# Walter0807/MotionBERT

Measured on AMD Instinct MI355X. Metric: clips/sec [B,243,17,3] DSTformer fwd+bwd, higher is better.
Workload: dtype bf16; 1 GPU; MotionBERT full DSTformer (dim_feat 512, depth 5, 8 heads, mlp_ratio 2) train step: fwd + bwd + AdamW, 64 clips/GPU x T=243 x J=17, random-init weights, pose loss (mpjpe + 0.5 n_mpjpe + 20 velocity, fused kernel), one-launch flat AdamW; global_batch=64, frames=243, parallelism=dp1

## Files before the change

include/mbx.h:

```cpp
#ifndef MBX_H
#define MBX_H
#include <stddef.h>
#include <stdint.h>

#ifdef __cplusplus
extern "C" {
#endif

enum mbx_dtype {
    MBX_F32 = 0,
    MBX_BF16 = 1,
    MBX_BF16_LO = 2
};

enum mbx_epilogue {
    MBX_EPI_STORE = 0,
    MBX_EPI_GELU  = 1,
    MBX_EPI_RESID = 2,
    MBX_EPI_TANH  = 3,
    MBX_EPI_DGELU = 4,
    MBX_EPI_LNBWD = 5,
    MBX_EPI_LNBWD_T = 9,
    MBX_EPI_GELU_D = 10,
    MBX_EPI_MULAUX = 11
};

enum mbx_attn_mode {
    MBX_ATTN_SPATIAL  = 0,
    MBX_ATTN_TEMPORAL = 1
};

const char* mbx_last_error(void);
int mbx_version(void);

int mbx_prep_weights(const int64_t* desc, int n_desc, int max_n, int max_k, int dtype, void* stream);

int mbx_embed_fwd(const float* x, const float* w, const float* b, const float* pos, const float* temp,
                  float* h, int B, int T, int J, int Din, int C, void* stream);
size_t mbx_embed_bwd_ws(int T, int J, int Din, int C);
int mbx_embed_bwd(const float* dh, const float* x, const float* w, float* dw, float* db, float* dpos,
                  float* dtemp, float* dx, int B, int T, int J, int Din, int C, void* ws, void* stream);
int mbx_embed_bwd_pair(const void* dh_a, const void* dh_b, const float* x, const float* w, float* dw, float* db, float* dpos,
                       float* dtemp, float* dx, int B, int T, int J, int Din, int C, void* ws, void* stream);

int mbx_layernorm_fwd(const float* x, const float* gamma, const float* beta, float eps, void* y,
                      float* mean, float* rstd, int M, int C, int dtype, void* stream);
size_t mbx_layernorm_bwd_ws(int C);
int mbx_layernorm_bwd(const void* dy, const float* x, const float* mean, const float* rstd, const float* gamma,
                      const float* dres, const float* extra, float* dx, void* dx_t, float* dgamma, float* dbeta,
                      int M, int C, int dtype, void* ws, void* stream);
int mbx_layernorm_bwd_planes(const float* dy, const float* x, const float* mean, const float* rstd, const float* gamma, const float* dres,
                             const float* extra, float* dx, void* dx_hi, void* dx_lo, float* dgamma, float* dbeta, int M, int C,
                             void* ws, void* stream);

int mbx_gemm_nt(const void* a, const void* w, const float* bias, int epilogue, void* out_t, void* out2_t,
                float* out_f, const float* resid, const void* aux_t, int M, int N, int K, int dtype, void* stream);
size_t mbx_gemm_tn_ws(int M, int N, int K);
int mbx_gemm_tn(const void* dy, const void* a, float* dw, float* db, int M, int N, int K, int dtype,
                void* ws, void* stream);

int mbx_fold_norm_weights(const int64_t* desc, int n_desc, int max_n, int max_k, void* stream);
int mbx_gemm_nt_dgelu_stats(const void* a, const void* w, void* out_t, const void* aux_t, const float* bias_f,
                            const float* rsum, float* part, int M, int N, int K, void* stream);
int mbx_gemm_nt_gelu_d(const void* a, const void* w, const float* bias, void* out_d, void* out_g, int M, int N, int K, void* stream);
int mbx_gemm_nt_mul(const void* a, const void* w, const void* aux, void* out, int M, int N, int K, void* stream);
int mbx_lnbwd_rowc(const float* part, int nb, const float* rstd, float* rowc, int M, int C, void* stream);
int mbx_gemm_nt_lnbwd(const void* a, const void* w, const void* xhat, const float* rowc, const float* dres,
                      const float* extra, float* dx, void* dx_t, int M, int N, int K, void* stream);
int mbx_gemm_nt_lnbwd_t(const void* a, const void* w, const void* xhat, const float* rowc, const void* dres_t,
                        const float* extra, float* dx, void* dx_t, int M, int N, int K, void* stream);
size_t mbx_unfold_norm_grads_ws(int N, int K);
int mbx_unfold_norm_grads(float* dw, const float* db, const float* w, const float* gamma, const float* beta,
                          float* dgamma, float* dbeta, int N, int K, void* ws, void* stream);

size_t mbx_mlp_pack_bytes(int C, int hidden);
int mbx_mlp_pack_weights(const void* w1, const void* w2, void* packed, int C, int hidden, void* stream);
int mbx_mlp_fused_fwd(const void* a, int raw_in, const void* packed, const float* b1, const float* b2, const float* rsum,
                      const float* resid, float* y, void* y_t, float eps, float* mean, float* rstd, int M, int C, int hidden,
                      void* stream);
size_t mbx_proj_mlp_pack_bytes(int C, int hidden);
int mbx_proj_mlp_pack_weights(const void* wp, const void* w1, const void* w2, void* packed, int C, int hidden, void* stream);
int mbx_proj_mlp_fused_fwd(const void* o, const void* packed, const float* bp, const float* b1, const float* b2, const float* rsum,
                           const float* resid, float* y, float eps, int M, int C, int hidden, void* stream);

size_t mbx_rows_pack_bytes(int N, int K);
int mbx_rows_pack_nk(const void* w, void* packed, int N, int K, void* stream);
int mbx_rows_gemm_nk(const void* a, const void* packed, const float* bias, const float* rsum, const float* mean, const float* rstd,
                     void* out, int M, int N, int K, void* stream);
int mbx_rows_gemm_nk_ln(const float* x, const void* packed, const float* bias, const float* rsum, float eps, void* out, int M, int N,
                        int K, void* stream);

int mbx_gelu_fwd(const void* u, void* g, size_t n, int dtype, void* stream);

int mbx_split_bf16(const float* x, void* hi, void* lo, size_t n, void* stream);
int mbx_gemm_nt_x3(const void* a_hi, const void* a_lo, const void* w_hi, const void* w_lo, const float* bias, int epilogue,
                   float* out_t, float* out2_t, float* out_f, const float* resid, const float* aux_t, int M, int N, int K,
                   void* stream);
int mbx_gemm_nt_x3p(const void* a_hi, const void* a_lo, const void* w_hi, const void* w_lo, const float* bias, int epilogue,
                    float* out_t, void* pl_hi, void* pl_lo, const float* aux_t, int M, int N, int K, void* stream);
int mbx_layernorm_fwd_planes(const float* x, const float* gamma, const float* beta, float eps, void* y_hi, void* y_lo, float* mean,
                             float* rstd, int M, int C, void* stream);
size_t mbx_gemm_tn_x3_workspace(int M, int N, int K);
int mbx_gemm_tn_x3(const void* dy_hi, const void* dy_lo, const void* a_hi, const void* a_lo, float* dw, float* db, int M,
                   int N, int K, void* ws, void* stream);

int mbx_attn_fwd(const void* qkv, void* o, float* lse, int B, int T, int J, int H, int hd, float scale,
                 int mode, int dtype, void* stream);
int mbx_attn_fwd_drop(const void* qkv, void* o, float* lse, int B, int T, int J, int H, int hd, float scale,
                      int mode, int dtype, float p, uint64_t seed, void* stream);
int mbx_attn_bwd(const void* qkv, const void* o, const void* d_o, const float* lse, void* dqkv, int B, int T,
                 int J, int H, int hd, float scale, int mode, int dtype, void* stream);
int mbx_attn_bwd_drop(const void* qkv, const void* o, const void* d_o, const float* lse, void* dqkv, int B, int T,
                      int J, int H, int hd, float scale, int mode, int dtype, float p, uint64_t seed, void* stream);
int mbx_attn_bwd_planes(const void* qkv, const void* o, const void* d_o, const float* lse, void* dqkv_hi, void* dqkv_lo, int B, int T,
                        int J, int H, int hd, float scale, int mode, float p, uint64_t seed, void* stream);
int mbx_attn_bwd_stats(const void* qkv, const void* o, const void* d_o, const float* lse, void* dqkv, const float* bias_f,
                       const float* rsum, float* part, int B, int T, int J, int H, int hd, float scale, int mode, void* stream);

int mbx_fuse_fwd(const float* x_st, const float* x_ts, const float* w, const float* b, float* out, float* alpha,
                 int M, int C, void* stream);
int mbx_fuse_ln_fwd(const float* x_st, const float* x_ts, const float* w, const float* b, float* out, float* alpha,
                    const float* g1, const float* b1, void* xn1, const float* g2, const float* b2, void* xn2, float eps,
                    float* mean, float* rstd, int M, int C, int dtype, void* stream);
size_t mbx_fuse_bwd_ws(int C);
int mbx_fuse_bwd(const float* dh, const float* x_st, const float* x_ts, const float* alpha, const float* w,
                 float* d_st, float* d_ts, void* d_st_t, void* d_ts_t, float* dw, float* db, int M, int C,
                 int dtype, void* ws, void* stream);
int mbx_fuse_bwd_pair(const void* dh_a, const void* dh_b, const float* x_st, const float* x_ts, const float* alpha, const float* w,
                      void* d_st_t, void* d_ts_t, float* dw, float* db, int M, int C, void* ws, void* stream);
int mbx_average(const float* x_st, const float* x_ts, float* out, size_t n, void* stream);
int mbx_average_bwd(const float* dh, float* d_st, float* d_ts, void* d_st_t, void* d_ts_t, size_t n, int dtype,
                    void* stream);

int mbx_head_fwd(const float* rep, const float* w, const float* b, float* out, int M, int R, int Dout, void* stream);
size_t mbx_head_bwd_ws(int R, int Dout);
int mbx_head_bwd(const float* dout, const float* rep, const float* w, void* dpre_t, float* dw, float* db,
                 int M, int R, int Dout, int dtype, void* ws, void* stream);
int mbx_tanh_bwd(const float* drep, const float* rep, void* dpre_t, size_t n, int dtype, void* stream);

size_t mbx_pose_loss_ws(int B, int T);
int mbx_pose_loss(const float* pred, const float* gt, float lambda_scale, float lambda_velocity, float* losses, float* dpred,
                  float grad_scale, int B, int T, int J, void* ws, void* stream);
size_t mbx_pose_loss_full_ws(int B, int T);
int mbx_pose_loss_full(const float* pred, const float* gt, float lambda_scale, float lambda_velocity, float lambda_lv, float lambda_lg,
                       float lambda_a, float lambda_av, float* losses, float* dpred, float grad_scale, int B, int T, int J, void* ws,
                       void* stream);
size_t mbx_loss_2d_weighted_ws(int B, int T);
int mbx_loss_2d_weighted(const float* pred, const float* target, int target_stride, const float* conf, int conf_stride, float* loss,
                         float* dpred, float grad_scale, int B, int T, int J, void* ws, void* stream);
int mbx_adamw_step(float* p, const float* g, float* m, float* v, size_t n, float* state, float beta1, float beta2, float eps,
                   float weight_decay, int tick, void* stream);

int mbx_pool_rep_fwd(const float* rep, float* pooled, int N, int Mp, int T, int J, int R, float p, uint64_t seed, void* stream);
int mbx_tanh_pool_bwd(const float* dpooled, const float* rep, void* dpre_t, int N, int Mp, int T, int J, int R, float p,
                      uint64_t seed, int dtype, void* stream);

int mbx_dropout(const void* x, void* y, size_t n, float p, uint64_t seed, int dtype, void* stream);
int mbx_residual_drop(float* y, const float* x, size_t rows, int C, int rows_per_sample, float p, uint64_t seed, float p_path,
                      uint64_t seed_path, void* stream);
int mbx_grad_drop(const float* dy, void* dy_t, size_t rows, int C, int rows_per_sample, float p, uint64_t seed, float p_path,
                  uint64_t seed_path, int dtype, void* stream);

int mbx_augment2d(const float* x, float* y, int B, int T, int J, int Cin, const float* noise_mean, const float* noise_std,
                  const float* noise_weight, float uniform_range, float jitter_std, float d2c_a, float d2c_b, float d2c_m,
                  float d2c_s, float mask_ratio, float mask_T_ratio, int flags, uint64_t seed, void* stream);
int mbx_embed_fwd_tta(const float* x, const int* perm, const float* w, const float* b, const float* pos, const float* temp,
                      float* h, int B, int T, int J, int Din, int C, void* stream);
int mbx_flip_average(const float* out2, const int* perm, float* out, int B, int T, int J, int D, void* stream);

int mbx_pose_errors(const float* pred, const float* gt, const float* hw, const float* factor, const float* x, int x_channels, int rootrel,
                    int gt_2d, double* e1, double* e2, int N, int T, int J, void* stream);
size_t mbx_eval_reduce_ws(int F, int A);
int mbx_eval_reduce(const double* e1, const double* e2, int n_err, const int* row_ptr, int n_row_ptr, const int* slots, int nnz,
                    const int* action, int F, int A, double* per_action, double* summary, int* count, void* ws, void* stream);

size_t mbx_rows_n_pack_bytes(int N, int K);
int mbx_rows_n_pack_many(const int64_t* desc, int n_desc, int N, int max_k, void* stream);
int mbx_rows_lnbwd_t(const void* dy, const void* packed, const void* xhat, const float* rstd, const void* dres_t, void* dx_t, int M,
                     int N, int K, void* stream);
int mbx_rows_resid_ln(const void* a, const void* packed, const float* bias, const float* resid, float* y, void* xhat, float* mean,
                      float* rstd, float eps, int M, int N, int K, void* stream);

size_t mbx_supcon_loss_ws(int A, int D);
int mbx_supcon_loss(const float* feat, const int* labels, int bsz, int n_views, int D, float temperature, float base_temperature,
                    int normalize, float grad_scale, float* loss, float* dfeat, void* ws, void* stream);
int mbx_nn_cosine(const float* anchors, const int* anchor_labels, int M, const float* test, const int* test_labels, int N, int D,
                  int* pred_label, float* best_sim, long long* hits, void* stream);

int mbx_rot6d_theta_fwd(const float* x6, float* rotmat, float* aa, int M, void* stream);
int mbx_rot6d_theta_bwd(const float* x6, const float* drotmat, const float* daa, float* dx6, int M, void* stream);
size_t mbx_mesh_param_loss_ws(int F);
// ... 93 lines not shown
```

motionbert_amd/csrc/elementwise.hip:

```cpp
#include "mbx_common.h"

static thread_local char g_err[512] = "";
int mbx_set_error(const char* fmt, ...) {
    va_list ap;
    va_start(ap, fmt);
    vsnprintf(g_err, sizeof(g_err), fmt, ap);
    va_end(ap);
    return 1;
}
extern "C" const char* mbx_last_error(void) { return g_err; }

#include <atomic>
static std::atomic<uintptr_t> g_lds_key[512];
static std::atomic<size_t> g_lds_size[512];
int mbx_set_dyn_lds(const void* kernel, size_t bytes, const char* who) {
    if (bytes > 160 * 1024) return mbx_set_error("%s: needs %zu bytes of LDS (> 160 KiB)", who, bytes);
    int dev = 0;
    if (hipGetDevice(&dev) != hipSuccess) dev = 0;
    const uintptr_t key = (reinterpret_cast<uintptr_t>(kernel) << 6) ^ (uintptr_t)(dev + 1);
    int slot = (int)((key * 0x9E3779B97F4A7C15ull) >> 55);
    for (int probe = 0; probe < 512; ++probe, slot = (slot + 1) & 511) {
        uintptr_t k = g_lds_key[slot].load(std::memory_order_acquire);
        if (k == 0 && g_lds_key[slot].compare_exchange_strong(k, key, std::memory_order_acq_rel)) k = key;
        if (k != key) continue;
        if (g_lds_size[slot].load(std::memory_order_acquire) >= bytes) return 0;
        const hipError_t e = hipFuncSetAttribute(kernel, hipFuncAttributeMaxDynamicSharedMemorySize, (int)bytes);
        if (e != hipSuccess) return mbx_set_error("%s: hipFuncSetAttribute(%zu): %s", who, bytes, hipGetErrorString(e));
        size_t cur = g_lds_size[slot].load(std::memory_order_relaxed);
        while (cur < bytes && !g_lds_size[slot].compare_exchange_weak(cur, bytes, std::memory_order_release)) { }
        return 0;
    }
    const hipError_t e = hipFuncSetAttribute(kernel, hipFuncAttributeMaxDynamicSharedMemorySize, (int)bytes);
    return e == hipSuccess ? 0 : mbx_set_error("%s: hipFuncSetAttribute(%zu): %s", who, bytes, hipGetErrorString(e));
}
static std::atomic<int> g_cus[64];
int mbx_cu_count() {
    int dev = 0;
    if (hipGetDevice(&dev) != hipSuccess || dev < 0 || dev >= 64) dev = 0;
    int c = g_cus[dev].load(std::memory_order_relaxed);
    if (c > 0) return c;
    if (hipDeviceGetAttribute(&c, hipDeviceAttributeMultiprocessorCount, dev) != hipSuccess || c <= 0) c = 256;
    g_cus[dev].store(c, std::memory_order_relaxed);
    return c;
}
extern "C" int mbx_version(void) { return 210; }

static inline int clamp_grid(size_t want, int cap) { return (int)(want < (size_t)cap ? (want ? want : 1) : (size_t)cap); }

__device__ __forceinline__ float4 ld4(const float* p) { return *reinterpret_cast<const float4*>(p); }
template <int CL>
__global__ __launch_bounds__(256) void colsum4_kernel(const float* __restrict__ part, int nparts, size_t stride, int ncols,
                                                      float* __restrict__ out0, float* __restrict__ out1, int split) {
    constexpr int PLW = 64 / CL, PL = 4 * PLW;
    __shared__ float4 red[PL][CL];
    const int lane = threadIdx.x & 63, wave = threadIdx.x >> 6;
    const int cl = lane % CL, pl = wave * PLW + lane / CL;
    const int c = (blockIdx.x * CL + cl) * 4;
    float4 a0 = make_float4(0.f, 0.f, 0.f, 0.f), a1 = a0, a2 = a0, a3 = a0;
    if (c < ncols) {
        const float* p = part + c;
        int i = pl;
        for (; i + 3 * PL < nparts; i += 4 * PL) {
            const float4 v0 = ld4(p + (size_t)i * stride), v1 = ld4(p + (size_t)(i + PL) * stride);
            const float4 v2 = ld4(p + (size_t)(i + 2 * PL) * stride), v3 = ld4(p + (size_t)(i + 3 * PL) * stride);
            a0 += v0; a1 += v1; a2 += v2; a3 += v3;
        }
        for (; i < nparts; i += PL) a0 += ld4(p + (size_t)i * stride);
    }
    red[pl][cl] = (a0 + a1) + (a2 + a3);
    __syncthreads();
    if (pl == 0 && c < ncols) {
        float4 t = red[0][cl];
#pragma unroll
        for (int q = 1; q < PL; ++q) t += red[q][cl];
        float* o = c < split ? out0 + c : out1 + (c - split);
        if ((reinterpret_cast<uintptr_t>(o) & 15) == 0) {
            *reinterpret_cast<float4*>(o) = t;
        } else {
            o[0] = t.x; o[1] = t.y; o[2] = t.z; o[3] = t.w;
        }
    }
}
__global__ __launch_bounds__(256) void colsum_kernel(const float* __restrict__ part, int nparts, int stride, int col0,
                                                     int ncols, float* __restrict__ out) {
    __shared__ float red[4][64];
    const int cl = threadIdx.x & 63, grp = threadIdx.x >> 6;
    const int c = blockIdx.x * 64 + cl;
    float s0 = 0.f, s1 = 0.f, s2 = 0.f, s3 = 0.f;
    if (c < ncols) {
        const float* p = part + col0 + c;
        int i = grp;
        for (; i + 12 < nparts; i += 16) {
            s0 += p[(size_t)i * stride];
            s1 += p[(size_t)(i + 4) * stride];
            s2 += p[(size_t)(i + 8) * stride];
            s3 += p[(size_t)(i + 12) * stride];
        }
        for (; i < nparts; i += 4) s0 += p[(size_t)i * stride];
    }
    red[grp][cl] = (s0 + s1) + (s2 + s3);
    __syncthreads();
    if (grp == 0 && c < ncols) out[c] = (red[0][cl] + red[1][cl]) + (red[2][cl] + red[3][cl]);
}
static int launch_colsum2(const float* part, int nparts, int stride, int col0, int ncols, float* out0, float* out1, int split,
                          hipStream_t s) {
    const bool vec = ncols % 4 == 0 && col0 % 4 == 0 && stride % 4 == 0 && split % 4 == 0 &&
                     (reinterpret_cast<uintptr_t>(part + col0) & 15) == 0;
    if (!vec) {
        hipLaunchKernelGGL(colsum_kernel, dim3((split + 63) / 64), dim3(256), 0, s, part, nparts, stride, col0, split, out0);
        if (ncols > split)
            hipLaunchKernelGGL(colsum_kernel, dim3((ncols - split + 63) / 64), dim3(256), 0, s, part, nparts, stride, col0 + split,
                               ncols - split, out1);
    } else if (ncols / 4 >= 64 * 512) {
        hipLaunchKernelGGL(colsum4_kernel<64>, dim3((ncols / 4 + 63) / 64), dim3(256), 0, s, part + col0, nparts, (size_t)stride, ncols,
                           out0, out1, split);
    } else {
        hipLaunchKernelGGL(colsum4_kernel<16>, dim3((ncols / 4 + 15) / 16), dim3(256), 0, s, part + col0, nparts, (size_t)stride, ncols,
                           out0, out1, split);
    }
    MBX_LAUNCH_CHECK("colsum");
    return 0;
}
int mbx_launch_colsum(const float* part, int nparts, int stride, int col0, int ncols, float* out, hipStream_t s) {
    return launch_colsum2(part, nparts, stride, col0, ncols, out, nullptr, ncols, s);
}

struct BfLo {};
template <> struct Cvt<BfLo> {
    static __device__ __forceinline__ bf16_t from_f(float v) { return f2bf(v - bf2f(f2bf(v))); }
};
template <typename T> struct PrepOut { typedef T type; };
template <> struct PrepOut<BfLo> { typedef bf16_t type; };
template <typename TT>
__global__ __launch_bounds__(256) void prep_weights_kernel(const int64_t* __restrict__ desc) {
    typedef typename PrepOut<TT>::type T;
    __shared__ float tile[32][33];
    const int64_t* d = desc + (size_t)blockIdx.y * 5;
    const float* src = reinterpret_cast<const float*>(d[0]);
    T* dst_n = reinterpret_cast<T*>(d[1]);
    T* dst_t = reinterpret_cast<T*>(d[2]);
    const int N = (int)d[3], K = (int)d[4];
    const int tk = (K + 31) / 32, tn = (N + 31) / 32;
    if ((int)blockIdx.x >= tk * tn) return;
    const int n0 = (blockIdx.x / tk) * 32, k0 = (blockIdx.x % tk) * 32;
    const int cx = threadIdx.x & 31, ry = threadIdx.x >> 5;
#pragma unroll
    for (int i = 0; i < 4; ++i) {
        const int r = ry + 8 * i;
        float v = 0.f;
        if (n0 + r < N && k0 + cx < K) {
            v = src[(size_t)(n0 + r) * K + k0 + cx];
            if (dst_n) dst_n[(size_t)(n0 + r) * K + k0 + cx] = Cvt<TT>::from_f(v);
        }
        tile[r][cx] = v;
    }
    __syncthreads();
    if (dst_t) {
#pragma unroll
        for (int i = 0; i < 4; ++i) {
            const int r = ry + 8 * i;
            if (k0 + r < K && n0 + cx < N) dst_t[(size_t)(k0 + r) * N + n0 + cx] = Cvt<TT>::from_f(tile[cx][r]);
        }
    }
}
extern "C" int mbx_prep_weights(const int64_t* desc, int n_desc, int max_n, int max_k, int dtype, void* stream) {
    MBX_CHECK_ARG(desc && n_desc > 0 && max_n > 0 && max_k > 0, "prep_weights: bad arguments");
    dim3 grid(((max_n + 31) / 32) * ((max_k + 31) / 32), n_desc);
    if (dtype == MBX_BF16)
        hipLaunchKernelGGL(prep_weights_kernel<bf16_t>, grid, dim3(256), 0, (hipStream_t)stream, desc);
    else if (dtype == MBX_F32)
        hipLaunchKernelGGL(prep_weights_kernel<float>, grid, dim3(256), 0, (hipStream_t)stream, desc);
    else if (dtype == MBX_BF16_LO)
        hipLaunchKernelGGL(prep_weights_kernel<BfLo>, grid, dim3(256), 0, (hipStream_t)stream, desc);
    else
        return mbx_set_error("prep_weights: unknown dtype %d", dtype);
    MBX_LAUNCH_CHECK("prep_weights");
    return 0;
}

template <typename T>
__global__ __launch_bounds__(256) void gelu_fwd_kernel(const T* __restrict__ u, T* __restrict__ g, size_t n4) {
    for (size_t i = (size_t)blockIdx.x * 256 + threadIdx.x; i < n4; i += (size_t)gridDim.x * 256) {
        float v[4];
        load4<T>(u + i * 4, v);
#pragma unroll
        for (int e = 0; e < 4; ++e) v[e] = gelu_erf(v[e]);
        store4<T>(g + i * 4, v);
    }
}
extern "C" int mbx_gelu_fwd(const void* u, void* g, size_t n, int dtype, void* stream) {
    MBX_CHECK_ARG(u && g && n % 4 == 0, "gelu_fwd: bad arguments");
    if (n == 0) return 0;
    const int grid = clamp_grid((n / 4 + 255) / 256, 256 * 16);
    if (dtype == MBX_BF16)
        hipLaunchKernelGGL(gelu_fwd_kernel<bf16_t>, dim3(grid), dim3(256), 0, (hipStream_t)stream, (const bf16_t*)u, (bf16_t*)g, n / 4);
    else if (dtype == MBX_F32)
        hipLaunchKernelGGL(gelu_fwd_kernel<float>, dim3(grid), dim3(256), 0, (hipStream_t)stream, (const float*)u, (float*)g, n / 4);
    else
        return mbx_set_error("gelu_fwd: unknown dtype %d", dtype);
    MBX_LAUNCH_CHECK("gelu_fwd");
    return 0;
}

__global__ __launch_bounds__(256) void split_bf16_kernel(const float* __restrict__ x, bf16_t* __restrict__ hi, bf16_t* __restrict__ lo,
                                                        size_t n4) {
    for (size_t idx = (size_t)blockIdx.x * 256 + threadIdx.x; idx < n4; idx += (size_t)gridDim.x * 256) {
        float v[4], h[4], l[4];
        load4<float>(x + idx * 4, v);
#pragma unroll
        for (int e = 0; e < 4; ++e) { h[e] = bf2f(f2bf(v[e])); l[e] = v[e] - h[e]; }
        store4<bf16_t>(hi + idx * 4, h);
        store4<bf16_t>(lo + idx * 4, l);
    }
}
extern "C" int mbx_split_bf16(const float* x, void* hi, void* lo, size_t n, void* stream) {
    MBX_CHECK_ARG(x && hi && lo, "split_bf16: null pointer");
    MBX_CHECK_ARG(n % 4 == 0, "split_bf16: n %% 4 != 0");
    if (n == 0) return 0;
    const int grid = clamp_grid((n / 4 + 255) / 256, 256 * 16);
    hipLaunchKernelGGL(split_bf16_kernel, dim3(grid), dim3(256), 0, (hipStream_t)stream, x, (bf16_t*)hi, (bf16_t*)lo, n / 4);
    MBX_LAUNCH_CHECK("split_bf16");
    return 0;
}

__global__ __launch_bounds__(256) void embed_fwd_kernel(const float* __restrict__ x, const float* __restrict__ w,
                                                        const float* __restrict__ b, const float* __restrict__ pos,
                                                        const float* __restrict__ temp, float* __restrict__ h, int M,
                                                        int T, int J, int Din, int C) {
    const int c4n = C >> 2;
    const size_t total = (size_t)M * c4n;
    for (size_t idx = (size_t)blockIdx.x * 256 + threadIdx.x; idx < total; idx += (size_t)gridDim.x * 256) {
        const int m = (int)(idx / c4n), c = (int)(idx % c4n) * 4;
        const int j = m % J, t = (m / J) % T;
        const float4 bb = *reinterpret_cast<const float4*>(b + c);
        const float4 pp = *reinterpret_cast<const float4*>(pos + (size_t)j * C + c);
        const float4 tt = *reinterpret_cast<const float4*>(temp + (size_t)t * C + c);
        float a0 = 0.f, a1 = 0.f, a2 = 0.f, a3 = 0.f;
        for (int k = 0; k < Din; ++k) {
            const float xv = x[(size_t)m * Din + k];
            a0 = fmaf(xv, w[(size_t)(c + 0) * Din + k], a0);
            a1 = fmaf(xv, w[(size_t)(c + 1) * Din + k], a1);
            a2 = fmaf(xv, w[(size_t)(c + 2) * Din + k], a2);
            a3 = fmaf(xv, w[(size_t)(c + 3) * Din + k], a3);
        }
        *reinterpret_cast<float4*>(h + (size_t)m * C + c) =
            make_float4(((a0 + bb.x) + pp.x) + tt.x, ((a1 + bb.y) + pp.y) + tt.y, ((a2 + bb.z) + pp.z) + tt.z,
                        ((a3 + bb.w) + pp.w) + tt.w);
    }
}
#define EMBF_MAXDIN 4
__global__ __launch_bounds__(256) void embed_fwd_rows_kernel(const float* __restrict__ x, const float* __restrict__ w,
                                                             const float* __restrict__ b, const float* __restrict__ pos,
                                                             const float* __restrict__ temp, float* __restrict__ h, int M,
                                                             int T, int J, int Din, int C, int chunk) {
    const int c4n = C >> 2, rpp = 256 / c4n;
    const int c = ((int)threadIdx.x % c4n) * 4, rsub = (int)threadIdx.x / c4n;
    float wv[4][EMBF_MAXDIN];
#pragma unroll
    for (int e = 0; e < 4; ++e)
#pragma unroll
        for (int k = 0; k < EMBF_MAXDIN; ++k) wv[e][k] = k < Din ? w[(size_t)(c + e) * Din + k] : 0.f;
    const float4 bb = *reinterpret_cast<const float4*>(b + c);
    const int end = min(M, ((int)blockIdx.x + 1) * chunk);
    int m = (int)blockIdx.x * chunk + rsub;
    int j = m % J, t = (m / J) % T;
    for (; m < end; m += 4 * rpp) {
        float xv[4][EMBF_MAXDIN];
        float4 pp[4], tt[4];
        int jj = j, tq = t;
#pragma unroll
        for (int u = 0; u < 4; ++u) {
            const int mu = min(m + u * rpp, M - 1);
#pragma unroll
            for (int k = 0; k < EMBF_MAXDIN; ++k) xv[u][k] = k < Din ? x[(size_t)mu * Din + k] : 0.f;
            pp[u] = *reinterpret_cast<const float4*>(pos + (size_t)jj * C + c);
            tt[u] = *reinterpret_cast<const float4*>(temp + (size_t)tq * C + c);
            jj += rpp;
            if (jj >= J) { jj -= J; tq = tq + 1 == T ? 0 : tq + 1; }
        }
#pragma unroll
        for (int u = 0; u < 4; ++u) {
            float a[4] = {0.f, 0.f, 0.f, 0.f};
#pragma unroll
            for (int k = 0; k < EMBF_MAXDIN; ++k)
                if (k < Din) {
#pragma unroll
                    for (int e = 0; e < 4; ++e) a[e] = fmaf(xv[u][k], wv[e][k], a[e]);
                }
            if (m + u * rpp < end)
                *reinterpret_cast<float4*>(h + (size_t)(m + u * rpp) * C + c) =
                    make_float4(((a[0] + bb.x) + pp[u].x) + tt[u].x, ((a[1] + bb.y) + pp[u].y) + tt[u].y,
                                ((a[2] + bb.z) + pp[u].z) + tt[u].z, ((a[3] + bb.w) + pp[u].w) + tt[u].w);
        }
        j = jj;
        t = tq;
    }
}
extern "C" int mbx_embed_fwd(const float* x, const float* w, const float* b, const float* pos, const float* temp,
                             float* h, int B, int T, int J, int Din, int C, void* stream) {
    MBX_CHECK_ARG(x && w && b && pos && temp && h, "embed_fwd: null pointer");
    MBX_CHECK_ARG(B > 0 && T > 0 && J > 0 && Din > 0 && C > 0 && C % 4 == 0, "embed_fwd: bad shape (C %% 4 != 0?)");
    const int M = B * T * J;
    const int c4n = C / 4;
    if (c4n >= 16 && c4n <= 256 && (c4n & (c4n - 1)) == 0 && Din <= EMBF_MAXDIN && 256 / c4n <= J) {
        const int rpp = 256 / c4n;
        const int blocks = clamp_grid((M + 4 * rpp - 1) / (4 * rpp), 256 * 8);
        int chunk = (M + blocks - 1) / blocks;
        chunk = ((chunk + 4 * rpp - 1) / (4 * rpp)) * (4 * rpp);
        const int grid = (M + chunk - 1) / chunk;
        hipLaunchKernelGGL(embed_fwd_rows_kernel, dim3(grid), dim3(256), 0, (hipStream_t)stream, x, w, b, pos, temp, h, M, T, J, Din, C, chunk);
    } else {
        const int grid = clamp_grid(((size_t)M * (C / 4) + 255) / 256, 256 * 16);
        hipLaunchKernelGGL(embed_fwd_kernel, dim3(grid), dim3(256), 0, (hipStream_t)stream, x, w, b, pos, temp, h, M, T, J, Din, C);
    }
    MBX_LAUNCH_CHECK("embed_fwd");
    return 0;
}

template <bool TTA>
__global__ __launch_bounds__(256) void embed_fwd_ragged_kernel(const float* __restrict__ x, const int* __restrict__ perm,
                                                               const float* __restrict__ w, const float* __restrict__ b,
                                                               const float* __restrict__ pos, const float* __restrict__ temp,
                                                               const int* __restrict__ frame_t, float* __restrict__ h, int F, int J,
                                                               int Din, int C, int n_temp) {
    const int c4n = C >> 2;
    const size_t rows = (size_t)(TTA ? 2 : 1) * F * J, total = rows * c4n;
    for (size_t idx = (size_t)blockIdx.x * 256 + threadIdx.x; idx < total; idx += (size_t)gridDim.x * 256) {
        const size_t mo = idx / c4n;
        const int c = (int)(idx % c4n) * 4;
        const int j = (int)(mo % J);
        size_t f = mo / J;
        const bool flip = TTA && f >= (size_t)F;
        if (flip) f -= F;
        const int t = frame_t[f];
        if (t < 0 || t >= n_temp) continue;
        const size_t ms = f * J + (flip ? perm[j] : j);
        const float4 bb = *reinterpret_cast<const float4*>(b + c);
        const float4 pp = *reinterpret_cast<const float4*>(pos + (size_t)j * C + c);
        const float4 tt = *reinterpret_cast<const float4*>(temp + (size_t)t * C + c);
        float a0 = 0.f, a1 = 0.f, a2 = 0.f, a3 = 0.f;
        for (int k = 0; k < Din; ++k) {
            float xv = x[ms * Din + k];
            if (flip && k == 0) xv = -xv;
            a0 = fmaf(xv, w[(size_t)(c + 0) * Din + k], a0);
            a1 = fmaf(xv, w[(size_t)(c + 1) * Din + k], a1);
            a2 = fmaf(xv, w[(size_t)(c + 2) * Din + k], a2);
            a3 = fmaf(xv, w[(size_t)(c + 3) * Din + k], a3);
        }
        *reinterpret_cast<float4*>(h + mo * C + c) =
            make_float4(((a0 + bb.x) + pp.x) + tt.x, ((a1 + bb.y) + pp.y) + tt.y, ((a2 + bb.z) + pp.z) + tt.z, ((a3 + bb.w) + pp.w) + tt.w);
    }
}
static int embed_fwd_ragged_impl(const char* who, const float* x, const int* perm, const float* w, const float* b, const float* pos,
                                 const float* temp, const int* frame_t, float* h, int F, int J, int Din, int C, int n_temp, bool tta,
                                 void* stream) {
    MBX_CHECK_ARG(x && w && b && pos && temp && frame_t && h && (!tta || perm), "%s: null pointer", who);
    MBX_CHECK_ARG(F > 0 && J > 0 && Din > 0 && C > 0 && C % 4 == 0 && n_temp > 0, "%s: bad shape (C %% 4 != 0?)", who);
    const int grid = clamp_grid(((size_t)(tta ? 2 : 1) * F * J * (C / 4) + 255) / 256, 256 * 16);
    if (tta)
        hipLaunchKernelGGL(embed_fwd_ragged_kernel<true>, dim3(grid), dim3(256), 0, (hipStream_t)stream, x, perm, w, b, pos, temp, frame_t, h, F, J,
                           Din, C, n_temp);
    else
        hipLaunchKernelGGL(embed_fwd_ragged_kernel<false>, dim3(grid), dim3(256), 0, (hipStream_t)stream, x, perm, w, b, pos, temp, frame_t, h, F, J,
                           Din, C, n_temp);
    MBX_LAUNCH_CHECK(who);
    return 0;
}
extern "C" int mbx_embed_fwd_ragged(const float* x, const float* w, const float* b, const float* pos, const float* temp, const int* frame_t,
                                    float* h, int F, int J, int Din, int C, int n_temp, void* stream) {
    return embed_fwd_ragged_impl("embed_fwd_ragged", x, nullptr, w, b, pos, temp, frame_t, h, F, J, Din, C, n_temp, false, stream);
}
extern "C" int mbx_embed_fwd_tta_ragged(const float* x, const int* perm, const float* w, const float* b, const float* pos, const float* temp,
                                        const int* frame_t, float* h, int F, int J, int Din, int C, int n_temp, void* stream) {
    return embed_fwd_ragged_impl("embed_fwd_tta_ragged", x, perm, w, b, pos, temp, frame_t, h, F, J, Din, C, n_temp, true, stream);
}

#define EMB_MAXDIN 4
__device__ __forceinline__ float4 embed_dh4(const float* __restrict__ dh, const bf16_t* __restrict__ dh_a, const bf16_t* __restrict__ dh_b, size_t o) {
    if (dh_a == nullptr) return *reinterpret_cast<const float4*>(dh + o);
    float u[4], v[4];
    load4<bf16_t>(dh_a + o, u);
    load4<bf16_t>(dh_b + o, v);
    return make_float4(u[0] + v[0], u[1] + v[1], u[2] + v[2], u[3] + v[3]);
}
__global__ __launch_bounds__(256) void embed_bwd_kernel(const float* __restrict__ dh, const float* __restrict__ x,
                                                        float* __restrict__ dtemp, float* __restrict__ part, int B, int T,
                                                        int J, int Din, int C, const bf16_t* __restrict__ dh_a = nullptr,
                                                        const bf16_t* __restrict__ dh_b = nullptr) {
    __shared__ float4 red[256][1 + EMB_MAXDIN];
    const int t = blockIdx.x;
    const int stride = J * C + C * Din + C;
    float* prow = part + (size_t)t * stride;
    const int nq = C / 4, ns = max(256 / nq, 1);
    for (int q0 = 0; q0 < nq; q0 += 256) {
        const int q = q0 + (int)threadIdx.x % min(nq, 256), sl = (int)threadIdx.x / min(nq, 256);
        const bool act = q < nq && sl < ns;
        const int c = q * 4;
        float4 at = make_float4(0.f, 0.f, 0.f, 0.f), aw[EMB_MAXDIN];
#pragma unroll
        for (int k = 0; k < EMB_MAXDIN; ++k) aw[k] = make_float4(0.f, 0.f, 0.f, 0.f);
        for (int j = 0; j < J; ++j) {
            float4 ap = make_float4(0.f, 0.f, 0.f, 0.f);
            if (act) {
                for (int b0 = sl; b0 < B; b0 += 8 * ns) {
                    float4 g[8];
#pragma unroll
                    for (int u = 0; u < 8; ++u) {
                        const int b = min(b0 + u * ns, B - 1);
                        g[u] = embed_dh4(dh, dh_a, dh_b, (((size_t)b * T + t) * J + j) * C + c);
                    }
#pragma unroll
                    for (int u = 0; u < 8; ++u) {
                        const int b = b0 + u * ns;
                        const float on = b < B ? 1.f : 0.f;
                        const size_t m = ((size_t)min(b, B - 1) * T + t) * J + j;
                        ap.x = fmaf(on, g[u].x, ap.x); ap.y = fmaf(on, g[u].y, ap.y); ap.z = fmaf(on, g[u].z, ap.z); ap.w = fmaf(on, g[u].w, ap.w);
#pragma unroll
                        for (int k = 0; k < EMB_MAXDIN; ++k)
                            if (k < Din) {
                                const float xv = on * x[m * Din + k];
                                aw[k].x = fmaf(g[u].x, xv, aw[k].x); aw[k].y = fmaf(g[u].y, xv, aw[k].y);
                                aw[k].z = fmaf(g[u].z, xv, aw[k].z); aw[k].w = fmaf(g[u].w, xv, aw[k].w);
                            }
                    }
                }
            }
            red[threadIdx.x][0] = ap;
            __syncthreads();
            if (act && sl == 0) {
                for (int s2 = 1; s2 < ns; ++s2) {
                    const float4 o = red[threadIdx.x + s2 * nq][0];
                    ap.x += o.x; ap.y += o.y; ap.z += o.z; ap.w += o.w;
                }
                *reinterpret_cast<float4*>(prow + (size_t)j * C + c) = ap;
                at.x += ap.x; at.y += ap.y; at.z += ap.z; at.w += ap.w;
            }
            __syncthreads();
        }
#pragma unroll
        for (int k = 0; k < EMB_MAXDIN; ++k) red[threadIdx.x][1 + k] = aw[k];
        __syncthreads();
        if (act && sl == 0) {
            *reinterpret_cast<float4*>(dtemp + (size_t)t * C + c) = at;
            *reinterpret_cast<float4*>(prow + (size_t)J * C + (size_t)C * Din + c) = at;
#pragma unroll
            for (int k = 0; k < EMB_MAXDIN; ++k)
                if (k < Din) {
                    float4 w4 = aw[k];
                    for (int s2 = 1; s2 < ns; ++s2) {
                        const float4 o = red[threadIdx.x + s2 * nq][1 + k];
                        w4.x += o.x; w4.y += o.y; w4.z += o.z; w4.w += o.w;
                    }
                    float* d = prow + (size_t)J * C + (size_t)c * Din + k;
                    d[0] = w4.x; d[Din] = w4.y; d[2 * Din] = w4.z; d[3 * Din] = w4.w;
                }
        }
        __syncthreads();
    }
}
__global__ __launch_bounds__(256) void embed_bwd_dx_kernel(const float* __restrict__ dh, const float* __restrict__ w,
                                                           float* __restrict__ dx, int M, int Din, int C,
                                                           const bf16_t* __restrict__ dh_a = nullptr, const bf16_t* __restrict__ dh_b = nullptr) {
    const int lane = threadIdx.x & 63;
    for (int m = blockIdx.x * 4 + (threadIdx.x >> 6); m < M; m += gridDim.x * 4) {
        float a[EMB_MAXDIN] = {0.f, 0.f, 0.f, 0.f};
        for (int c = lane; c < C; c += 64) {
            const float g = dh_a == nullptr ? dh[(size_t)m * C + c] : bf2f(dh_a[(size_t)m * C + c]) + bf2f(dh_b[(size_t)m * C + c]);
#pragma unroll
            for (int k = 0; k < EMB_MAXDIN; ++k)
                if (k < Din) a[k] = fmaf(g, w[(size_t)c * Din + k], a[k]);
        }
#pragma unroll
        for (int k = 0; k < EMB_MAXDIN; ++k) {
            const float s = wave_sum(a[k]);
            if (lane == 0 && k < Din) dx[(size_t)m * Din + k] = s;
        }
    }
}
extern "C" size_t mbx_embed_bwd_ws(int T, int J, int Din, int C) { return (size_t)T * ((size_t)J * C + (size_t)C * Din + C) * sizeof(float); }
static int launch_embed_bwd(const float* dh, const bf16_t* dh_a, const bf16_t* dh_b, const float* x, const float* w, float* dw, float* db,
                            float* dpos, float* dtemp, float* dx, int B, int T, int J, int Din, int C, void* ws, void* stream) {
    MBX_CHECK_ARG((dh || (dh_a && dh_b)) && x && w && dw && db && dpos && dtemp && ws, "embed_bwd: null pointer");
    MBX_CHECK_ARG(Din <= EMB_MAXDIN, "embed_bwd: dim_in %d > %d unsupported", Din, EMB_MAXDIN);
    MBX_CHECK_ARG(B > 0 && T > 0 && J > 0 && C > 0 && C % 4 == 0, "embed_bwd: bad shape (C %% 4 != 0?)");
    hipStream_t s = (hipStream_t)stream;
    float* part = (float*)ws;
    const int stride = J * C + C * Din + C;
    hipLaunchKernelGGL(embed_bwd_kernel, dim3(T), dim3(256), 0, s, dh, x, dtemp, part, B, T, J, Din, C, dh_a, dh_b);
    MBX_LAUNCH_CHECK("embed_bwd");
    if (mbx_launch_colsum(part, T, stride, 0, J * C, dpos, s)) return 1;
    if (mbx_launch_colsum(part, T, stride, J * C, C * Din, dw, s)) return 1;
    if (mbx_launch_colsum(part, T, stride, J * C + C * Din, C, db, s)) return 1;
    if (dx) {
        const int M = B * T * J;
        hipLaunchKernelGGL(embed_bwd_dx_kernel, dim3(clamp_grid((M + 3) / 4, 2048)), dim3(256), 0, s, dh, w, dx, M, Din, C, dh_a, dh_b);
        MBX_LAUNCH_CHECK("embed_bwd_dx");
    }
    return 0;
}
extern "C" int mbx_embed_bwd(const float* dh, const float* x, const float* w, float* dw, float* db, float* dpos,
                             float* dtemp, float* dx, int B, int T, int J, int Din, int C, void* ws, void* stream) {
    MBX_CHECK_ARG(dh, "embed_bwd: null pointer");
    return launch_embed_bwd(dh, nullptr, nullptr, x, w, dw, db, dpos, dtemp, dx, B, T, J, Din, C, ws, stream);
}
extern "C" int mbx_embed_bwd_pair(const void* dh_a, const void* dh_b, const float* x, const float* w, float* dw, float* db, float* dpos,
                                  float* dtemp, float* dx, int B, int T, int J, int Din, int C, void* ws, void* stream) {
    MBX_CHECK_ARG(dh_a && dh_b, "embed_bwd_pair: null pointer");
    return launch_embed_bwd(nullptr, (const bf16_t*)dh_a, (const bf16_t*)dh_b, x, w, dw, db, dpos, dtemp, dx, B, T, J, Din, C, ws, stream);
}

#define ROW_LOOP(k) _Pragma("unroll") for (int k = 0; k < VPL; ++k)
#define ROW_C(k) (((k) * 64 + lane) * 4)

static inline int vpl_for(int C) { return C <= 256 ? 1 : C <= 512 ? 2 : C <= 1024 ? 4 : C <= 2048 ? 8 : 0; }
#define DISPATCH_VPL(vpl, ...)           \
    switch (vpl) {                       \
        case 1: { constexpr int VPL = 1; __VA_ARGS__; } break; \
        case 2: { constexpr int VPL = 2; __VA_ARGS__; } break; \
        case 4: { constexpr int VPL = 4; __VA_ARGS__; } break; \
        case 8: { constexpr int VPL = 8; __VA_ARGS__; } break; \
        default: return mbx_set_error("row kernel: channel count unsupported (need C %% 4 == 0 and C <= 2048)"); \
    }

#define LN_BLOCKS 1024
template <typename T> struct Raw4;
template <> struct Raw4<float> {
    typedef float4 type;
    static __device__ __forceinline__ void unpack(const float4& r, float (&v)[4]) { v[0] = r.x; v[1] = r.y; v[2] = r.z; v[3] = r.w; }
};
template <> struct Raw4<bf16_t> {
    typedef uint2 type;
    static __device__ __forceinline__ void unpack(const uint2& r, float (&v)[4]) {
        v[0] = __uint_as_float(r.x << 16); v[1] = __uint_as_float(r.x & 0xffff0000u);
        v[2] = __uint_as_float(r.y << 16); v[3] = __uint_as_float(r.y & 0xffff0000u);
    }
};
__device__ __forceinline__ void unpack4(const float4& r, float (&v)[4]) { v[0] = r.x; v[1] = r.y; v[2] = r.z; v[3] = r.w; }

template <int VPL, bool FULL>
__device__ __forceinline__ void ln_fwd_load(const float* __restrict__ x, int row, int C, int lane, float4 (&raw)[VPL]) {
    ROW_LOOP(k) {
        const int c = ROW_C(k);
        raw[k] = make_float4(0.f, 0.f, 0.f, 0.f);
        if (FULL || c < C) raw[k] = ld4(x + (size_t)row * C + c);
    }
}
template <typename T, int VPL, bool FULL>
__device__ __forceinline__ void ln_fwd_row(const float4 (&raw)[VPL], const float (&g)[VPL][4], const float (&bt)[VPL][4], float eps,
                                           float invC, T* __restrict__ y, float* __restrict__ mean, float* __restrict__ rstd,
                                           int row, int C, int lane, bf16_t* __restrict__ y_lo = nullptr) {
    float v[VPL][4];
    float s = 0.f;
    ROW_LOOP(k) {
        unpack4(raw[k], v[k]);
        s += (v[k][0] + v[k][1]) + (v[k][2] + v[k][3]);
    }
    const float mu = wave_sum(s) * invC;
    float q = 0.f;
    ROW_LOOP(k) {
        const int c = ROW_C(k);
        if (FULL || c < C) {
#pragma unroll
            for (int i = 0; i < 4; ++i) { v[k][i] -= mu; q = fmaf(v[k][i], v[k][i], q); }
        }
    }
    const float rs = 1.0f / sqrtf(wave_sum(q) * invC + eps);
    ROW_LOOP(k) {
        const int c = ROW_C(k);
        if (FULL || c < C) {
            float o[4];
#pragma unroll
            for (int i = 0; i < 4; ++i) o[i] = fmaf(v[k][i] * rs, g[k][i], bt[k][i]);
            if (sizeof(T) == 4 && y_lo)
                store4_planes(reinterpret_cast<bf16_t*>(y) + (size_t)row * C + c, y_lo + (size_t)row * C + c, o);
            else
                store4<T>(y + (size_t)row * C + c, o);
        }
    }
    if (lane == 0) { mean[row] = mu; rstd[row] = rs; }
}
template <typename T, int VPL, bool FULL>
__global__ __launch_bounds__(256) void ln_fwd_kernel(const float* __restrict__ x, const float* __restrict__ gamma,
                                                     const float* __restrict__ beta, float eps, T* __restrict__ y,
                                                     float* __restrict__ mean, float* __restrict__ rstd, int M, int C,
                                                     bf16_t* __restrict__ y_lo) {
    const int lane = threadIdx.x & 63;
    float g[VPL][4], bt[VPL][4];
    ROW_LOOP(k) {
        const int c = ROW_C(k);
#pragma unroll
        for (int i = 0; i < 4; ++i) { g[k][i] = 0.f; bt[k][i] = 0.f; }
        if (gamma == nullptr) {
#pragma unroll
            for (int i = 0; i < 4; ++i) g[k][i] = 1.f;
        } else if (FULL || c < C) { load4<float>(gamma + c, g[k]); load4<float>(beta + c, bt[k]); }
    }
    const float invC = 1.0f / (float)C;
    const int step = gridDim.x * 4;
    for (int row0 = blockIdx.x * 4 + (threadIdx.x >> 6); row0 < M; row0 += 2 * step) {
        const int row1 = row0 + step;
        float4 ra[VPL], rb[VPL];
        ln_fwd_load<VPL, FULL>(x, row0, C, lane, ra);
        if (row1 < M) ln_fwd_load<VPL, FULL>(x, row1, C, lane, rb);
        ln_fwd_row<T, VPL, FULL>(ra, g, bt, eps, invC, y, mean, rstd, row0, C, lane, y_lo);
        if (row1 < M) ln_fwd_row<T, VPL, FULL>(rb, g, bt, eps, invC, y, mean, rstd, row1, C, lane, y_lo);
    }
}
#define LN_FWD_LAUNCH(TT, FULLV)                                                                                             \
    DISPATCH_VPL(vpl, hipLaunchKernelGGL((ln_fwd_kernel<TT, VPL, FULLV>), dim3(grid), dim3(256), 0, s, x, gamma, beta, eps, (TT*)y, \
                                         mean, rstd, M, C, (bf16_t*)y_lo))
static int launch_layernorm_fwd(const float* x, const float* gamma, const float* beta, float eps, void* y, void* y_lo, float* mean,
                                float* rstd, int M, int C, int dtype, void* stream);
extern "C" int mbx_layernorm_fwd(const float* x, const float* gamma, const float* beta, float eps, void* y, float* mean,
                                 float* rstd, int M, int C, int dtype, void* stream) {
    return launch_layernorm_fwd(x, gamma, beta, eps, y, nullptr, mean, rstd, M, C, dtype, stream);
}
extern "C" int mbx_layernorm_fwd_planes(const float* x, const float* gamma, const float* beta, float eps, void* y_hi, void* y_lo,
                                        float* mean, float* rstd, int M, int C, void* stream) {
    MBX_CHECK_ARG(y_lo, "layernorm_fwd_planes: null pointer");
    return launch_layernorm_fwd(x, gamma, beta, eps, y_hi, y_lo, mean, rstd, M, C, MBX_F32, stream);
}
static int launch_layernorm_fwd(const float* x, const float* gamma, const float* beta, float eps, void* y, void* y_lo, float* mean,
                                float* rstd, int M, int C, int dtype, void* stream) {
    MBX_CHECK_ARG(x && y && mean && rstd, "layernorm_fwd: null pointer");
    MBX_CHECK_ARG((gamma && beta) || (!gamma && !beta), "layernorm_fwd: gamma and beta come together (both NULL = plain normalisation)");
    MBX_CHECK_ARG(M > 0 && C > 0 && C % 4 == 0, "layernorm_fwd: bad shape M=%d C=%d", M, C);
    MBX_CHECK_ARG(dtype == MBX_BF16 || dtype == MBX_F32, "layernorm_fwd: unknown dtype %d", dtype);
    const int grid = clamp_grid((M + 3) / 4, LN_BLOCKS);
    const int vpl = vpl_for(C);
    const bool full = vpl > 0 && C == vpl * 256;
    hipStream_t s = (hipStream_t)stream;
    if (dtype == MBX_BF16) {
        if (full) { LN_FWD_LAUNCH(bf16_t, true); } else { LN_FWD_LAUNCH(bf16_t, false); }
    } else {
        if (full) { LN_FWD_LAUNCH(float, true); } else { LN_FWD_LAUNCH(float, false); }
    }
    MBX_LAUNCH_CHECK("layernorm_fwd");
    return 0;
}

__device__ __forceinline__ void block_fold_store(const float* lds , int n, float* __restrict__ dst) {
    for (int i = threadIdx.x; i < n; i += 256) dst[i] = (lds[i] + lds[n + i]) + (lds[2 * n + i] + lds[3 * n + i]);
}

template <typename T, int VPL, bool FULL, bool RES>
__device__ __forceinline__ void ln_bwd_load(const T* __restrict__ dy, const float* __restrict__ x, const float* __restrict__ dres,
                                            const float* __restrict__ mean, const float* __restrict__ rstd, int row, int C, int lane,
                                            typename Raw4<T>::type (&rd)[VPL], float4 (&rx)[VPL], float4 (&rr)[VPL], float& mu,
                                            float& rs) {
    mu = mean[row];
    rs = rstd[row];
    ROW_LOOP(k) {
        const int c = ROW_C(k);
        if (FULL || c < C) {
            const size_t o = (size_t)row * C + c;
            rd[k] = *reinterpret_cast<const typename Raw4<T>::type*>(dy + o);
            rx[k] = ld4(x + o);
            if (RES) rr[k] = ld4(dres + o);
        }
    }
}
template <typename T, int VPL, bool FULL, bool RES>
__device__ __forceinline__ void ln_bwd_row(const typename Raw4<T>::type (&rd)[VPL], const float4 (&rx)[VPL], const float4 (&rr)[VPL],
                                           float mu, float rs, const float (&g)[VPL][4], float (&ag)[VPL][4], float (&ab)[VPL][4],
                                           float invC, const float* __restrict__ extra, float* __restrict__ dx, T* __restrict__ dx_t,
                                           int row, int C, int lane, bf16_t* __restrict__ dx_lo = nullptr) {
    float d[VPL][4], xh[VPL][4];
    float s1 = 0.f, s2 = 0.f;
    ROW_LOOP(k) {
        const int c = ROW_C(k);
        if (FULL || c < C) {
            Raw4<T>::unpack(rd[k], d[k]);
            unpack4(rx[k], xh[k]);
#pragma unroll
            for (int i = 0; i < 4; ++i) {
                xh[k][i] = (xh[k][i] - mu) * rs;
                ag[k][i] = fmaf(d[k][i], xh[k][i], ag[k][i]);
                ab[k][i] += d[k][i];
                d[k][i] *= g[k][i];
                s1 += d[k][i];
                s2 = fmaf(d[k][i], xh[k][i], s2);
            }
        }
    }
    s1 = wave_sum(s1) * invC;
    s2 = wave_sum(s2) * invC;
    ROW_LOOP(k) {
        const int c = ROW_C(k);
        if (FULL || c < C) {
            float r[4];
#pragma unroll
            for (int i = 0; i < 4; ++i) r[i] = rs * (d[k][i] - s1 - xh[k][i] * s2);
            if (RES) {
                float t[4];
                unpack4(rr[k], t);
#pragma unroll
                for (int i = 0; i < 4; ++i) r[i] += t[i];
            }
            if (extra) {
                float t[4];
                load4<float>(extra + (size_t)row * C + c, t);
#pragma unroll
                for (int i = 0; i < 4; ++i) r[i] += t[i];
            }
            store4<float>(dx + (size_t)row * C + c, r);
            if (sizeof(T) == 4 && dx_lo)
                store4_planes(reinterpret_cast<bf16_t*>(dx_t) + (size_t)row * C + c, dx_lo + (size_t)row * C + c, r);
            else if (dx_t) store4<T>(dx_t + (size_t)row * C + c, r);
        }
    }
}
template <typename T, int VPL, bool FULL, bool RES>
__global__ __launch_bounds__(256) void ln_bwd_kernel(const T* __restrict__ dy, const float* __restrict__ x,
                                                     const float* __restrict__ mean, const float* __restrict__ rstd,
                                                     const float* __restrict__ gamma, const float* __restrict__ dres,
                                                     const float* __restrict__ extra, float* __restrict__ dx,
                                                     T* __restrict__ dx_t, float* __restrict__ part, int M, int C,
                                                     bf16_t* __restrict__ dx_lo) {
    extern __shared__ __attribute__((aligned(16))) float lds[];
    const int lane = threadIdx.x & 63, wave = threadIdx.x >> 6;
    float g[VPL][4], ag[VPL][4], ab[VPL][4];
    ROW_LOOP(k) {
        const int c = ROW_C(k);
#pragma unroll
        for (int i = 0; i < 4; ++i) { ag[k][i] = 0.f; ab[k][i] = 0.f; g[k][i] = 0.f; }
        if (FULL || c < C) load4<float>(gamma + c, g[k]);
    }
    const float invC = 1.0f / (float)C;
    const int step = gridDim.x * 4;
    for (int row0 = blockIdx.x * 4 + wave; row0 < M; row0 += 2 * step) {
        const int row1 = row0 + step;
        typename Raw4<T>::type da[VPL], db[VPL];
        float4 xa[VPL], xb[VPL], ra[VPL], rb[VPL];
        float mua, rsa, mub, rsb;
        ln_bwd_load<T, VPL, FULL, RES>(dy, x, dres, mean, rstd, row0, C, lane, da, xa, ra, mua, rsa);
        if (row1 < M) ln_bwd_load<T, VPL, FULL, RES>(dy, x, dres, mean, rstd, row1, C, lane, db, xb, rb, mub, rsb);
        ln_bwd_row<T, VPL, FULL, RES>(da, xa, ra, mua, rsa, g, ag, ab, invC, extra, dx, dx_t, row0, C, lane, dx_lo);
        if (row1 < M) ln_bwd_row<T, VPL, FULL, RES>(db, xb, rb, mub, rsb, g, ag, ab, invC, extra, dx, dx_t, row1, C, lane, dx_lo);
    }
    float* mine = lds + (size_t)wave * 2 * C;
    ROW_LOOP(k) {
        const int c = ROW_C(k);
        if (FULL || c < C) { store4<float>(mine + c, ag[k]); store4<float>(mine + C + c, ab[k]); }
    }
    __syncthreads();
    block_fold_store(lds, 2 * C, part + (size_t)blockIdx.x * 2 * C);
}
#define LN_BWD_LAUNCH(TT, FULLV, RESV)                                                                                        \
    DISPATCH_VPL(vpl, hipLaunchKernelGGL((ln_bwd_kernel<TT, VPL, FULLV, RESV>), dim3(grid), dim3(256), shm, s, (const TT*)dy, x, mean, \
                                         rstd, gamma, dres, extra, dx, (TT*)dx_t, part, M, C, (bf16_t*)dx_lo))
#define LN_BWD_LAUNCH_T(TT)                                                            \
    if (full && dres) { LN_BWD_LAUNCH(TT, true, true); }                               \
    else if (full) { LN_BWD_LAUNCH(TT, true, false); }                                 \
    else if (dres) { LN_BWD_LAUNCH(TT, false, true); }                                 \
    else { LN_BWD_LAUNCH(TT, false, false); }
extern "C" size_t mbx_layernorm_bwd_ws(int C) { return (size_t)LN_BLOCKS * 2 * C * sizeof(float); }
static int launch_layernorm_bwd(const void* dy, const float* x, const float* mean, const float* rstd, const float* gamma,
                                const float* dres, const float* extra, float* dx, void* dx_t, void* dx_lo, float* dgamma, float* dbeta,
                                int M, int C, int dtype, void* ws, void* stream);
extern "C" int mbx_layernorm_bwd(const void* dy, const float* x, const float* mean, const float* rstd, const float* gamma,
                                 const float* dres, const float* extra, float* dx, void* dx_t, float* dgamma, float* dbeta,
                                 int M, int C, int dtype, void* ws, void* stream) {
    return launch_layernorm_bwd(dy, x, mean, rstd, gamma, dres, extra, dx, dx_t, nullptr, dgamma, dbeta, M, C, dtype, ws, stream);
}
extern "C" int mbx_layernorm_bwd_planes(const float* dy, const float* x, const float* mean, const float* rstd, const float* gamma,
                                        const float* dres, const float* extra, float* dx, void* dx_hi, void* dx_lo, float* dgamma,
                                        float* dbeta, int M, int C, void* ws, void* stream) {
    MBX_CHECK_ARG(dx_hi && dx_lo, "layernorm_bwd_planes: null pointer");
    return launch_layernorm_bwd(dy, x, mean, rstd, gamma, dres, extra, dx, dx_hi, dx_lo, dgamma, dbeta, M, C, MBX_F32, ws, stream);
}
static int launch_layernorm_bwd(const void* dy, const float* x, const float* mean, const float* rstd, const float* gamma,
                                const float* dres, const float* extra, float* dx, void* dx_t, void* dx_lo, float* dgamma, float* dbeta,
                                int M, int C, int dtype, void* ws, void* stream) {
    MBX_CHECK_ARG(dy && x && mean && rstd && gamma && dx && dgamma && dbeta && ws, "layernorm_bwd: null pointer");
    MBX_CHECK_ARG(M > 0 && C > 0 && C % 4 == 0, "layernorm_bwd: bad shape M=%d C=%d", M, C);
    MBX_CHECK_ARG(dtype == MBX_BF16 || dtype == MBX_F32, "layernorm_bwd: unknown dtype %d", dtype);
    const int grid = clamp_grid((M + 3) / 4, LN_BLOCKS);
    const size_t shm = (size_t)4 * 2 * C * sizeof(float);
    const int vpl = vpl_for(C);
    const bool full = vpl > 0 && C == vpl * 256;
    hipStream_t s = (hipStream_t)stream;
    float* part = (float*)ws;
    if (dtype == MBX_BF16) {
        LN_BWD_LAUNCH_T(bf16_t)
    } else {
        LN_BWD_LAUNCH_T(float)
    }
    MBX_LAUNCH_CHECK("layernorm_bwd");
    return launch_colsum2(part, grid, 2 * C, 0, 2 * C, dgamma, dbeta, C, s);
}
// ... 303 lines not shown
        for (int i = 0; i < 4; ++i) { g0s[k][i] = g0t[k][i] = g1s[k][i] = g1t[k][i] = 0.f; w0s[k][i] = w0t[k][i] = w1s[k][i] = w1t[k][i] = 0.f; }
        if (c < C) {
            load4<float>(w + c, w0s[k]); load4<float>(w + C + c, w0t[k]);
            load4<float>(w + 2 * C + c, w1s[k]); load4<float>(w + 3 * C + c, w1t[k]);
        }
    }
    for (int row = blockIdx.x * 4 + wave; row < M; row += gridDim.x * 4) {
        const float a0 = alpha[(size_t)row * 2], a1 = alpha[(size_t)row * 2 + 1];
        float d[VPL][4], a[VPL][4], t[VPL][4];
        float da0 = 0.f, da1 = 0.f;
        ROW_LOOP(k) {
            const int c = ROW_C(k);
            if (c < C) {
                if (dh_a != nullptr) {
                    float e[4];
                    load4<bf16_t>(dh_a + (size_t)row * C + c, d[k]);
                    load4<bf16_t>(dh_b + (size_t)row * C + c, e);
#pragma unroll
                    for (int i = 0; i < 4; ++i) d[k][i] += e[i];
                } else {
                    load4<float>(dh + (size_t)row * C + c, d[k]);
                }
                load4<float>(x_st + (size_t)row * C + c, a[k]);
                load4<float>(x_ts + (size_t)row * C + c, t[k]);
#pragma unroll
                for (int i = 0; i < 4; ++i) { da0 = fmaf(d[k][i], a[k][i], da0); da1 = fmaf(d[k][i], t[k][i], da1); }
            }
        }
        da0 = wave_sum(da0);
        da1 = wave_sum(da1);
        const float dot = da0 * a0 + da1 * a1;
        const float dl0 = a0 * (da0 - dot), dl1 = a1 * (da1 - dot);
        gb0 += dl0;
        gb1 += dl1;
        ROW_LOOP(k) {
            const int c = ROW_C(k);
            if (c < C) {
                float rs[4], rt[4];
#pragma unroll
                for (int i = 0; i < 4; ++i) {
                    rs[i] = fmaf(d[k][i], a0, fmaf(dl0, w0s[k][i], dl1 * w1s[k][i]));
                    rt[i] = fmaf(d[k][i], a1, fmaf(dl0, w0t[k][i], dl1 * w1t[k][i]));
                    g0s[k][i] = fmaf(dl0, a[k][i], g0s[k][i]);
                    g0t[k][i] = fmaf(dl0, t[k][i], g0t[k][i]);
                    g1s[k][i] = fmaf(dl1, a[k][i], g1s[k][i]);
                    g1t[k][i] = fmaf(dl1, t[k][i], g1t[k][i]);
                }
                if (d_st != nullptr) {
                    store4<float>(d_st + (size_t)row * C + c, rs);
                    store4<float>(d_ts + (size_t)row * C + c, rt);
                }
                store4<T>(d_st_t + (size_t)row * C + c, rs);
                store4<T>(d_ts_t + (size_t)row * C + c, rt);
            }
        }
    }
    float* mine = lds + (size_t)wave * n;
    ROW_LOOP(k) {
        const int c = ROW_C(k);
        if (c < C) {
            store4<float>(mine + c, g0s[k]); store4<float>(mine + C + c, g0t[k]);
            store4<float>(mine + 2 * C + c, g1s[k]); store4<float>(mine + 3 * C + c, g1t[k]);
        }
    }
    if (lane == 0) { mine[4 * C] = gb0; mine[4 * C + 1] = gb1; mine[4 * C + 2] = 0.f; mine[4 * C + 3] = 0.f; }
    __syncthreads();
    block_fold_store(lds, n, part + (size_t)blockIdx.x * n);
}
extern "C" size_t mbx_fuse_bwd_ws(int C) { return (size_t)FUSE_BWD_BLOCKS * (4 * (size_t)C + 4) * sizeof(float); }
extern "C" int mbx_fuse_bwd(const float* dh, const float* x_st, const float* x_ts, const float* alpha, const float* w,
                            float* d_st, float* d_ts, void* d_st_t, void* d_ts_t, float* dw, float* db, int M, int C,
                            int dtype, void* ws, void* stream) {
    MBX_CHECK_ARG(dh && x_st && x_ts && alpha && w && d_st_t && d_ts_t && dw && db && ws, "fuse_bwd: null pointer");
    MBX_CHECK_ARG((d_st && d_ts) || (!d_st && !d_ts), "fuse_bwd: d_st and d_ts come together (both NULL: only the T-typed copies are written)");
    MBX_CHECK_ARG(M > 0 && C > 0 && C % 4 == 0, "fuse_bwd: bad shape");
    const int grid = clamp_grid((M + 3) / 4, FUSE_BWD_BLOCKS);
    const int n = 4 * C + 4;
    const size_t shm = (size_t)4 * n * sizeof(float);
    hipStream_t s = (hipStream_t)stream;
    float* part = (float*)ws;
    if (dtype == MBX_BF16) {
        DISPATCH_VPL(vpl_for(C), hipLaunchKernelGGL((fuse_bwd_kernel<bf16_t, VPL>), dim3(grid), dim3(256), shm, s, dh, x_st, x_ts, alpha, w, d_st, d_ts, (bf16_t*)d_st_t, (bf16_t*)d_ts_t, part, M, C));
    } else if (dtype == MBX_F32) {
        DISPATCH_VPL(vpl_for(C), hipLaunchKernelGGL((fuse_bwd_kernel<float, VPL>), dim3(grid), dim3(256), shm, s, dh, x_st, x_ts, alpha, w, d_st, d_ts, (float*)d_st_t, (float*)d_ts_t, part, M, C));
    } else {
        return mbx_set_error("fuse_bwd: unknown dtype %d", dtype);
    }
    MBX_LAUNCH_CHECK("fuse_bwd");
    if (mbx_launch_colsum(part, grid, n, 0, 4 * C, dw, s)) return 1;
    if (mbx_launch_colsum(part, grid, n, 4 * C, 2, db, s)) return 1;
    return 0;
}

extern "C" int mbx_fuse_bwd_pair(const void* dh_a, const void* dh_b, const float* x_st, const float* x_ts, const float* alpha, const float* w,
                                 void* d_st_t, void* d_ts_t, float* dw, float* db, int M, int C, void* ws, void* stream) {
    MBX_CHECK_ARG(dh_a && dh_b && x_st && x_ts && alpha && w && d_st_t && d_ts_t && dw && db && ws, "fuse_bwd_pair: null pointer");
    MBX_CHECK_ARG(M > 0 && C > 0 && C % 4 == 0, "fuse_bwd_pair: bad shape");
    const int grid = clamp_grid((M + 3) / 4, FUSE_BWD_BLOCKS);
    const int n = 4 * C + 4;
    const size_t shm = (size_t)4 * n * sizeof(float);
    hipStream_t s = (hipStream_t)stream;
    float* part = (float*)ws;
    DISPATCH_VPL(vpl_for(C), hipLaunchKernelGGL((fuse_bwd_kernel<bf16_t, VPL>), dim3(grid), dim3(256), shm, s, (const float*)nullptr, x_st, x_ts, alpha, w,
                                                (float*)nullptr, (float*)nullptr, (bf16_t*)d_st_t, (bf16_t*)d_ts_t, part, M, C, (const bf16_t*)dh_a, (const bf16_t*)dh_b));
    MBX_LAUNCH_CHECK("fuse_bwd_pair");
    if (mbx_launch_colsum(part, grid, n, 0, 4 * C, dw, s)) return 1;
    if (mbx_launch_colsum(part, grid, n, 4 * C, 2, db, s)) return 1;
    return 0;
}

__global__ __launch_bounds__(256) void average_kernel(const float* __restrict__ a, const float* __restrict__ b,
                                                      float* __restrict__ out, size_t n4) {
    for (size_t i = (size_t)blockIdx.x * 256 + threadIdx.x; i < n4; i += (size_t)gridDim.x * 256) {
        const float4 u = reinterpret_cast<const float4*>(a)[i], v = reinterpret_cast<const float4*>(b)[i];
        reinterpret_cast<float4*>(out)[i] = make_float4((u.x + v.x) * 0.5f, (u.y + v.y) * 0.5f, (u.z + v.z) * 0.5f, (u.w + v.w) * 0.5f);
    }
}
template <typename T>
__global__ __launch_bounds__(256) void average_bwd_kernel(const float* __restrict__ dh, float* __restrict__ d_st,
                                                          float* __restrict__ d_ts, T* __restrict__ d_st_t,
                                                          T* __restrict__ d_ts_t, size_t n4) {
    for (size_t i = (size_t)blockIdx.x * 256 + threadIdx.x; i < n4; i += (size_t)gridDim.x * 256) {
        float v[4];
        load4<float>(dh + i * 4, v);
#pragma unroll
        for (int k = 0; k < 4; ++k) v[k] *= 0.5f;
        store4<float>(d_st + i * 4, v);
        store4<float>(d_ts + i * 4, v);
        store4<T>(d_st_t + i * 4, v);
        store4<T>(d_ts_t + i * 4, v);
    }
}
extern "C" int mbx_average(const float* x_st, const float* x_ts, float* out, size_t n, void* stream) {
    MBX_CHECK_ARG(x_st && x_ts && out && n % 4 == 0, "average: bad arguments");
    hipLaunchKernelGGL(average_kernel, dim3(clamp_grid((n / 4 + 255) / 256, 4096)), dim3(256), 0, (hipStream_t)stream, x_st, x_ts, out, n / 4);
    MBX_LAUNCH_CHECK("average");
    return 0;
}
extern "C" int mbx_average_bwd(const float* dh, float* d_st, float* d_ts, void* d_st_t, void* d_ts_t, size_t n,
                               int dtype, void* stream) {
    MBX_CHECK_ARG(dh && d_st && d_ts && d_st_t && d_ts_t && n % 4 == 0, "average_bwd: bad arguments");
    const int grid = clamp_grid((n / 4 + 255) / 256, 4096);
    if (dtype == MBX_BF16)
        hipLaunchKernelGGL(average_bwd_kernel<bf16_t>, dim3(grid), dim3(256), 0, (hipStream_t)stream, dh, d_st, d_ts, (bf16_t*)d_st_t, (bf16_t*)d_ts_t, n / 4);
    else if (dtype == MBX_F32)
        hipLaunchKernelGGL(average_bwd_kernel<float>, dim3(grid), dim3(256), 0, (hipStream_t)stream, dh, d_st, d_ts, (float*)d_st_t, (float*)d_ts_t, n / 4);
    else
        return mbx_set_error("average_bwd: unknown dtype %d", dtype);
    MBX_LAUNCH_CHECK("average_bwd");
    return 0;
}

#define HEAD_MAXD 8
template <int VPL>
__global__ __launch_bounds__(256) void head_fwd_kernel(const float* __restrict__ rep, const float* __restrict__ w,
                                                       const float* __restrict__ b, float* __restrict__ out, int M, int R,
                                                       int Dout) {
    const int lane = threadIdx.x & 63;
    for (int row = blockIdx.x * 4 + (threadIdx.x >> 6); row < M; row += gridDim.x * 4) {
        float v[VPL][4];
        ROW_LOOP(k) {
            const int c = ROW_C(k);
            if (c < R) load4<float>(rep + (size_t)row * R + c, v[k]);
        }
        float mine = 0.f;
        for (int i = 0; i < Dout; ++i) {
            float a = 0.f;
            ROW_LOOP(k) {
                const int c = ROW_C(k);
                if (c < R) {
                    float ww[4];
                    load4<float>(w + (size_t)i * R + c, ww);
#pragma unroll
                    for (int e = 0; e < 4; ++e) a = fmaf(v[k][e], ww[e], a);
                }
            }
            a = wave_sum(a) + b[i];
            if (lane == i) mine = a;
        }
        if (lane < Dout) out[(size_t)row * Dout + lane] = mine;
    }
}
extern "C" int mbx_head_fwd(const float* rep, const float* w, const float* b, float* out, int M, int R, int Dout,
                            void* stream) {
    MBX_CHECK_ARG(rep && w && b && out, "head_fwd: null pointer");
    MBX_CHECK_ARG(M > 0 && R % 4 == 0 && Dout >= 1 && Dout <= HEAD_MAXD, "head_fwd: need R %% 4 == 0 and 1 <= dim_out <= %d", HEAD_MAXD);
    const int grid = clamp_grid((M + 3) / 4, 256 * 8);
    hipStream_t s = (hipStream_t)stream;
    DISPATCH_VPL(vpl_for(R), hipLaunchKernelGGL((head_fwd_kernel<VPL>), dim3(grid), dim3(256), 0, s, rep, w, b, out, M, R, Dout));
    MBX_LAUNCH_CHECK("head_fwd");
    return 0;
}

#define HEAD_BWD_BLOCKS 1024
template <typename T, int VPL>
__global__ __launch_bounds__(256) void head_bwd_kernel(const float* __restrict__ dout, const float* __restrict__ rep,
                                                       const float* __restrict__ w, T* __restrict__ dpre,
                                                       float* __restrict__ part, int M, int R, int Dout) {
    extern __shared__ __attribute__((aligned(16))) float lds[];
    const int lane = threadIdx.x & 63, wave = threadIdx.x >> 6;
    const int n = Dout * R + 8;
    float* mine = lds + (size_t)wave * n;
    constexpr int DG = 4;
    for (int i0 = 0; i0 < Dout; i0 += DG) {
        float gw[DG][VPL][4], gbv[DG];
#pragma unroll
        for (int j = 0; j < DG; ++j) {
            gbv[j] = 0.f;
            ROW_LOOP(k) {
#pragma unroll
                for (int e = 0; e < 4; ++e) gw[j][k][e] = 0.f;
            }
        }
        for (int row = blockIdx.x * 4 + wave; row < M; row += gridDim.x * 4) {
            float dvg[DG];
#pragma unroll
            for (int j = 0; j < DG; ++j) dvg[j] = i0 + j < Dout ? dout[(size_t)row * Dout + i0 + j] : 0.f;
#pragma unroll
            for (int j = 0; j < DG; ++j) gbv[j] += dvg[j];
            float dv[HEAD_MAXD];
            if (i0 == 0) {
#pragma unroll
                for (int q = 0; q < HEAD_MAXD; ++q) dv[q] = q < DG ? dvg[q < DG ? q : 0] : (q < Dout ? dout[(size_t)row * Dout + q] : 0.f);
            }
            ROW_LOOP(k) {
                const int c = ROW_C(k);
                if (c < R) {
                    float r[4];
                    load4<float>(rep + (size_t)row * R + c, r);
#pragma unroll
                    for (int j = 0; j < DG; ++j)
#pragma unroll
                        for (int e = 0; e < 4; ++e) gw[j][k][e] = fmaf(dvg[j], r[e], gw[j][k][e]);
                    if (i0 == 0) {
                        float o[4] = {0.f, 0.f, 0.f, 0.f};
#pragma unroll
                        for (int q = 0; q < HEAD_MAXD; ++q) {
                            if (q < Dout) {
                                float ww[4];
                                load4<float>(w + (size_t)q * R + c, ww);
#pragma unroll
                                for (int e = 0; e < 4; ++e) o[e] = fmaf(dv[q], ww[e], o[e]);
                            }
                        }
#pragma unroll
                        for (int e = 0; e < 4; ++e) o[e] *= (1.0f - r[e] * r[e]);
                        store4<T>(dpre + (size_t)row * R + c, o);
                    }
                }
            }
        }
#pragma unroll
        for (int j = 0; j < DG; ++j) {
            if (i0 + j < Dout) {
                ROW_LOOP(k) {
                    const int c = ROW_C(k);
                    if (c < R) store4<float>(mine + (size_t)(i0 + j) * R + c, gw[j][k]);
                }
                if (lane == 0) mine[Dout * R + i0 + j] = gbv[j];
            }
        }
    }
    if (lane == 0)
        for (int q = Dout; q < 8; ++q) mine[Dout * R + q] = 0.f;
    __syncthreads();
    block_fold_store(lds, n, part + (size_t)blockIdx.x * n);
}
extern "C" size_t mbx_head_bwd_ws(int R, int Dout) { return (size_t)HEAD_BWD_BLOCKS * ((size_t)Dout * R + 8) * sizeof(float); }
extern "C" int mbx_head_bwd(const float* dout, const float* rep, const float* w, void* dpre_t, float* dw, float* db,
                            int M, int R, int Dout, int dtype, void* ws, void* stream) {
    MBX_CHECK_ARG(dout && rep && w && dpre_t && dw && db && ws, "head_bwd: null pointer");
    MBX_CHECK_ARG(M > 0 && R % 4 == 0 && Dout >= 1 && Dout <= HEAD_MAXD, "head_bwd: need R %% 4 == 0 and 1 <= dim_out <= %d", HEAD_MAXD);
    const int grid = clamp_grid((M + 3) / 4, HEAD_BWD_BLOCKS);
    const int n = Dout * R + 8;
    const size_t shm = (size_t)4 * n * sizeof(float);
    MBX_CHECK_ARG(shm <= 160 * 1024, "head_bwd: dim_out*dim_rep too large for the LDS fold");
    hipStream_t s = (hipStream_t)stream;
    float* part = (float*)ws;
    if (dtype == MBX_BF16) {
        DISPATCH_VPL(vpl_for(R), hipLaunchKernelGGL((head_bwd_kernel<bf16_t, VPL>), dim3(grid), dim3(256), shm, s, dout, rep, w, (bf16_t*)dpre_t, part, M, R, Dout));
    } else if (dtype == MBX_F32) {
        DISPATCH_VPL(vpl_for(R), hipLaunchKernelGGL((head_bwd_kernel<float, VPL>), dim3(grid), dim3(256), shm, s, dout, rep, w, (float*)dpre_t, part, M, R, Dout));
    } else {
        return mbx_set_error("head_bwd: unknown dtype %d", dtype);
    }
    MBX_LAUNCH_CHECK("head_bwd");
    if (mbx_launch_colsum(part, grid, n, 0, Dout * R, dw, s)) return 1;
    if (mbx_launch_colsum(part, grid, n, Dout * R, Dout, db, s)) return 1;
    return 0;
}

template <typename T>
__global__ __launch_bounds__(256) void tanh_bwd_kernel(const float* __restrict__ drep, const float* __restrict__ rep,
                                                       T* __restrict__ dpre, size_t n4) {
    for (size_t i = (size_t)blockIdx.x * 256 + threadIdx.x; i < n4; i += (size_t)gridDim.x * 256) {
        float d[4], r[4];
        load4<float>(drep + i * 4, d);
        load4<float>(rep + i * 4, r);
#pragma unroll
        for (int k = 0; k < 4; ++k) d[k] *= (1.0f - r[k] * r[k]);
        store4<T>(dpre + i * 4, d);
    }
}
extern "C" int mbx_tanh_bwd(const float* drep, const float* rep, void* dpre_t, size_t n, int dtype, void* stream) {
    MBX_CHECK_ARG(drep && rep && dpre_t && n % 4 == 0, "tanh_bwd: bad arguments");
    const int grid = clamp_grid((n / 4 + 255) / 256, 4096);
    if (dtype == MBX_BF16)
        hipLaunchKernelGGL(tanh_bwd_kernel<bf16_t>, dim3(grid), dim3(256), 0, (hipStream_t)stream, drep, rep, (bf16_t*)dpre_t, n / 4);
    else if (dtype == MBX_F32)
        hipLaunchKernelGGL(tanh_bwd_kernel<float>, dim3(grid), dim3(256), 0, (hipStream_t)stream, drep, rep, (float*)dpre_t, n / 4);
    else
        return mbx_set_error("tanh_bwd: unknown dtype %d", dtype);
    MBX_LAUNCH_CHECK("tanh_bwd");
    return 0;
}
```

motionbert_amd/engine.py:

```python
from __future__ import annotations

from collections import namedtuple
from dataclasses import dataclass
from typing import Any, ClassVar, Dict, List, Optional

import os

import torch

EPI_STORE = 0
EPI_GELU = 1
EPI_RESID = 2
EPI_TANH = 3
EPI_DGELU = 4

MODE_SPATIAL = 0
MODE_TEMPORAL = 1


@dataclass(frozen=True)
class ModelCfg:
    dim_in: int
    dim_out: int
    C: int
# ... 132 lines not shown
        self.rows_lnbwd = sw.rows_lnbwd and self._can('can_rows_lnbwd')
        self.Pn: Dict[str, torch.Tensor] = {}
        self.rows_resid_ln = sw.rows_resid_ln and self._can('can_rows_resid_ln')
        self.Pf: Dict[str, torch.Tensor] = {}
        self.block_grad_t = sw.block_grad_t and self.rows_lnbwd and hasattr(ops, 'fuse_bwd_pair') and hasattr(ops, 'embed_bwd_pair')
        self.gelu_d = sw.gelu_d and self.rows_lnbwd and self._can('can_gelu_d')
        self.rawln = False
        self.rawln_allowed = sw.rawln
        self.Pk: Dict[str, torch.Tensor] = {}
        self.Pk_proj: Dict[str, str] = {}
        self.proj_mlp = sw.proj_mlp and hasattr(ops, 'proj_mlp_fused_fwd')

    def _choose_row_kernels(self):
        cfg = self.cfg
        self.lnbwd_rows = bool(self.rows_lnbwd and rows_lnbwd_fits(self.M, cfg.C, max(3 * cfg.C, cfg.hidden)))
        self.resid_rows = bool(self.rows_resid_ln and rows_resid_ln_fits(self.M, cfg.C, max(cfg.C, cfg.hidden)))

    def _streams(self):
        if not (self.dual and self.dev.type == 'cuda'):
            return None, None
        idx = self.dev.index if self.dev.index is not None else torch.cuda.current_device()
        side = Engine._side_streams.get(idx)
        if side is None:
            side = Engine._side_streams[idx] = torch.cuda.Stream(device=idx)
        return torch.cuda.current_stream(idx), side

    def _f(self, *shape):
        return torch.empty(shape, dtype=torch.float32, device=self.dev)

    def _t(self, *shape):
        return torch.empty(shape, dtype=self.T, device=self.dev)

    def _can(self, name: str) -> bool:
        return bool(getattr(self.ops, name, lambda *_: False)(self.T, self.cfg))

    @staticmethod
    def _await(extra):
        return extra() if callable(extra) else extra

    def _drops(self, pre: str, sub: int) -> Optional[Drops]:
        if self.drop_seed is None:
            return None
        from .dropmask import site_seed
        cfg = self.cfg
        stream, level = (0 if pre.startswith('blocks_st') else 1), int(pre.split('.')[1])
        pp = float(cfg.dpr[level]) if cfg.dpr else 0.0
        if cfg.drop <= 0 and pp <= 0 and cfg.attn_drop <= 0:
            return None
        ss = lambda kind: site_seed(self.drop_seed, level, stream, sub, kind)
        return Drops(cfg.drop, ss(1), ss(2), pp, ss(3), cfg.attn_drop, ss(0))

    def _xn(self, sv, pre, norm):
        return sv['xn'] if sv['xn'] is not None else self._mm(self._layernorm(sv['x'], f'{pre}.{norm}')[0])

    def _layernorm(self, x, norm):
        xn, mean, rstd = self._op(self.M, self.cfg.C), self._f(self.M), self._f(self.M)
        self.ops.layernorm_fwd(x, self.P[norm + '.weight'] if norm else None, self.P[norm + '.bias'] if norm else None, self.cfg.eps, xn, mean, rstd)
        return xn, mean, rstd

    def _norm_in(self, x, pre, norm, ln):
        xn, mean, rstd = ln if ln is not None else self._layernorm(x, None if self.fold else f'{pre}.{norm}')
        return self._mm(xn), mean, rstd

    def _mm(self, t):
        return self.ops.split(t) if self.x3 and not isinstance(t, tuple) else t

    def _op(self, *shape):
        if self.x3 and self.x3_planes:
            return (torch.empty(shape, dtype=torch.bfloat16, device=self.dev), torch.empty(shape, dtype=torch.bfloat16, device=self.dev))
        return self._t(*shape)

    def _weight_cache_key(self, need_grad: bool):
        if need_grad or not hasattr(self.ops, 'weight_cache') or self.dev.type != 'cuda' or torch.cuda.is_current_stream_capturing():
            return None
        return (tuple((p.data_ptr(), p._version) for p in self.P.values()), self.T, self.fold, self.rawln, self.proj_mlp, self.x3, self.resid_rows)

    def prepare_weights(self, need_grad: bool):
        cfg, ops, P = self.cfg, self.ops, self.P
        self._choose_row_kernels()
        if need_grad and hasattr(ops, 'weight_cache') and self.dev.type == 'cuda':
            ops.weight_cache.pop(self.dev.index, None)
        key = self._weight_cache_key(need_grad)
        if key is not None:
            hit = ops.weight_cache.get(self.dev.index)
            if hit is not None and hit[0] == key and len(hit[1]) == len(P) and all(r() is p for r, p in zip(hit[1], P.values())):
                self.Wn, self.Wt, self.Bf, self.Rs, self.Pk, self.Pk_proj, self.Pf = hit[2]
                return
        self._prepare_weights(need_grad)
        if key is not None:
            import weakref
            ops.weight_cache[self.dev.index] = (key, [weakref.ref(p) for p in P.values()], (self.Wn, self.Wt, self.Bf, self.Rs, self.Pk, self.Pk_proj, self.Pf))

    def _prepare_weights(self, need_grad: bool):
        cfg, ops, P = self.cfg, self.ops, self.P
        if self.fold:
            pairs = folded_pairs(cfg)
            folded = {l for l, _ in pairs}
            self.Wn, self.Wt = ops.prep_weights(P, [n for n in linear_names(cfg) if n not in folded], self.T, need_grad)
            fn, ft, self.Bf, self.Rs = ops.fold_norm_weights(P, pairs, need_grad, self.T)
            self.Wn.update(fn)
            self.Wt.update(ft)
            if self.resid_rows and not self.rawln:
                lins = [f'{pre}.{mod}.{LINEARS[typ][1]}' for pre, _, sub, typ, _, mod, _ in sublayers(cfg) if sub < 3]
                self.Pf = dict(zip(lins, ops.rows_n_pack_many([self.Wn[lin] for lin in lins])))
            if need_grad and self.lnbwd_rows and self.gstream_allowed:
                first = {f'{pre}.{mod}.qkv' for pre, _, sub, _, _, mod, _ in sublayers(cfg) if sub == 0 and not (self.block_grad_t and cfg.att_fuse)}
                lins = [lin for lin, _ in pairs if lin not in first]
                self.Pn = dict(zip(lins, ops.rows_n_pack_many([ft[lin] for lin in lins])))
            if self.rawln:
                before = None
                for blk, _, sub, typ, _, m, _ in sublayers(cfg):
                    pre = f'{blk}.{m}'
                    if typ == 'mlp' and self.proj_mlp and before is not None and before[0] == 'attn':
                        self.Pk_proj[pre] = f'{blk}.{before[1]}.proj'
                        self.Pk[pre] = ops.proj_mlp_pack_weights(self.Wn[self.Pk_proj[pre]], self.Wn[pre + '.fc1'], self.Wn[pre + '.fc2'])
                    elif typ == 'mlp':
                        self.Pk[pre] = ops.mlp_pack_weights(self.Wn[pre + '.fc1'], self.Wn[pre + '.fc2'])
                    before = (typ, m) if sub < 3 else None
                    for a in ('attn_s', 'attn_t') if sub == 3 else ():
                        self.Pk[f'{blk}.{a}.qkv'] = ops.rows_pack_nk(self.Wn[f'{blk}.{a}.qkv'])
        else:
            self.Wn, self.Wt = ops.prep_weights(P, linear_names(cfg), self.T, need_grad, x3=self.x3)

    def forward(self, x: torch.Tensor, return_rep, need_grad: bool, tta_perm=None, ragged=None):
        cfg, ops, P = self.cfg, self.ops, self.P
        pool = return_rep if isinstance(return_rep, tuple) else None
        return_rep = bool(return_rep)
        self.dev = x.device
        B, T, J, Din = x.shape
        self.ragged = None
        if ragged is not None:
            if need_grad or self.drop_seed is not None or pool is not None:
                raise RuntimeError('a ragged batch is an inference path: no gradient, no dropout and no pooled representation')
            clip_tab, frame_t, n_clips, max_len = ragged
            if B != 1 or frame_t.numel() != T or clip_tab.numel() != 2 * n_clips or not 1 <= n_clips <= T:
                raise RuntimeError(f'a ragged batch is x [1,F,J,C] with frame_t [F] and clip_tab [n_clips,2]: got x {tuple(x.shape)}, frame_t '
                                   f'{tuple(frame_t.shape)}, clip_tab {tuple(clip_tab.shape)} for {n_clips} clips')
            if not 1 <= max_len <= min(cfg.maxlen, 256):
                raise RuntimeError(f'a ragged batch takes clips of 1 .. {min(cfg.maxlen, 256)} frames, got max_len = {max_len}')
            if 2 * T * max(cfg.H, J) >= 1 << 31:
                raise RuntimeError(f'a ragged batch of {T} frames is too large')
            if tta_perm is not None:
                clip_tab = clip_tab.reshape(n_clips, 2).repeat(2, 1)
                clip_tab[n_clips:, 0] += T
                n_clips = 2 * n_clips
            self.ragged = (clip_tab.contiguous(), n_clips, int(max_len))
        if tta_perm is not None:
            B = 2 * B
        M, C = B * T * J, cfg.C
        self.B, self.Tlen, self.M = B, T, M
        self.rawln = not need_grad and self.fold and self.drop_seed is None and self.rawln_allowed and self._can('can_fuse_mlp')
        self.prepare_weights(need_grad)
        h = self._f(M, C)
        if ragged is not None and tta_perm is not None:
            ops.embed_fwd_tta_ragged(x, tta_perm, P['joints_embed.weight'], P['joints_embed.bias'], P['pos_embed'], P['temp_embed'], frame_t, h, T, J)
        elif ragged is not None:
            ops.embed_fwd_ragged(x, P['joints_embed.weight'], P['joints_embed.bias'], P['pos_embed'], P['temp_embed'], frame_t, h, T, J)
        elif tta_perm is not None:
            ops.embed_fwd_tta(x, tta_perm, P['joints_embed.weight'], P['joints_embed.bias'], P['pos_embed'], P['temp_embed'], h, B // 2, T, J)
        else:
            ops.embed_fwd(x, P['joints_embed.weight'], P['joints_embed.bias'], P['pos_embed'], P['temp_embed'], h, B, T, J)
        if self.drop_seed is not None and cfg.drop > 0:
            from .dropmask import site_seed
            ops.dropout(h, h, cfg.drop, site_seed(self.drop_seed, -1, 0, 0, 1))
        saved: Dict[str, Any] = dict(x=x, levels=[], return_rep=return_rep)
        main, side = self._streams()
        fuse_ln = cfg.att_fuse and hasattr(ops, 'fuse_ln_fwd')
        ln_st = ln_ts = ln_tail = None
        if self.fold and not self.rawln:
            ln_st = ln_ts = self._layernorm(h, None)
        for i in range(cfg.depth):
            if side is not None:
                side.wait_stream(main)
                with torch.cuda.stream(side):
                    x_ts, sv_ts = self._block_fwd(h, f'blocks_ts.{i}', 'ts', need_grad, ln_ts)
                x_st, sv_st = self._block_fwd(h, f'blocks_st.{i}', 'st', need_grad, ln_st)
                main.wait_stream(side)
            else:
                x_st, sv_st = self._block_fwd(h, f'blocks_st.{i}', 'st', need_grad, ln_st)
                x_ts, sv_ts = self._block_fwd(h, f'blocks_ts.{i}', 'ts', need_grad, ln_ts)
            ln_st = ln_ts = None
            hn = self._f(M, C)
            if fuse_ln and not (self.rawln and i + 1 < cfg.depth):
                alpha, mean, rstd = self._f(M, 2), self._f(M), self._f(M)
                last = i + 1 == cfg.depth
                n1, n2 = (('norm', None) if last else (None, None) if self.fold else
                          (f"blocks_st.{i + 1}.{ORDER['st'][0][1]}", f"blocks_ts.{i + 1}.{ORDER['ts'][0][1]}"))
                xn1, xn2 = self._t(M, C), (self._t(M, C) if n2 else None)
                gb = [P[f'{n}.{k}'] if n else None for n in (n1, n2) for k in ('weight', 'bias')]
                ops.fuse_ln_fwd(x_st, x_ts, P[f'ts_attn.{i}.weight'], P[f'ts_attn.{i}.bias'], hn, alpha,
                                gb[0], gb[1], xn1, gb[2], gb[3], xn2, cfg.eps, mean, rstd)
                if last:
                    ln_tail = (xn1, mean, rstd)
                else:
                    ln_st, ln_ts = (xn1, mean, rstd), (xn2 if n2 else xn1, mean, rstd)
            elif cfg.att_fuse:
                alpha = self._f(M, 2)
                ops.fuse_fwd(x_st, x_ts, P[f'ts_attn.{i}.weight'], P[f'ts_attn.{i}.bias'], hn, alpha)
            else:
                alpha = None
                ops.average(x_st, x_ts, hn)
            if need_grad:
                saved['levels'].append(dict(st=sv_st, ts=sv_ts, x_st=x_st, x_ts=x_ts, alpha=alpha))
            h = hn
        if ln_tail is not None:
            xn, mean, rstd = ln_tail
        else:
            xn, mean, rstd = self._layernorm(h, 'norm')
        xn = self._mm(xn)
        rep4 = self._f(B, T, J, cfg.R)
        rep = rep4.view(M, cfg.R)
        ops.gemm_nt(xn, self.Wn['pre_logits.fc'], P['pre_logits.fc.bias'], EPI_TANH, out_f=rep)
        if need_grad:
            saved.update(h=h, xn=xn, mean=mean, rstd=rstd, rep=rep, pool=pool)
        if pool is not None:
            _, persons, p_drop, seed = pool
            if B % persons:
                raise RuntimeError(f'pooled representation: batch {B} is not a multiple of persons={persons}')
            out = self._f(B // persons, J, cfg.R)
            ops.pool_rep_fwd(rep, out, B // persons, persons, T, J, p_drop, seed)
        elif return_rep:
            out = rep4
        else:
            out = self._f(B, T, J, cfg.dim_out)
            ops.head_fwd(rep, P['head.weight'], P['head.bias'], out.view(M, cfg.dim_out))
            if tta_perm is not None:
                both, out = out, self._f(B // 2, T, J, cfg.dim_out)
                ops.flip_average(both, tta_perm, out)
        return out, saved

    def _block_fwd(self, x, pre, kind, need_grad, ln=None):
        svs = []
        order = ORDER[kind]
        pend = None
        for sub, (typ, norm, mod, mode) in enumerate(order):
            nxt = order[sub + 1][1] if sub + 1 < len(order) else None
            if typ == 'attn':
                defer = self.rawln and self.proj_mlp and sub + 1 < len(order) and order[sub + 1][0] == 'mlp'
                x, sv, ln, pend = self._attn_fwd(x, pre, norm, mod, mode, need_grad, sub, ln, nxt, defer_proj=defer)
            else:
                x, sv, ln = self._mlp_fwd(x, pre, norm, mod, need_grad, sub, ln, nxt, pending_proj=pend)
                pend = None
            svs.append(sv)
        assert pend is None, 'an attention deferred its proj to an MLP that never came'
        return x, svs

    def _resid_gemm(self, a, lin, x, dm, pre, nxt):
        cfg, ops, P = self.cfg, self.ops, self.P
        y = self._f(self.M, cfg.C)
        drop = dm is not None and dm.branch
        if self.fold and nxt is not None and lin in self.Pf and self.resid_rows and not drop:
            xn, mean, rstd = self._op(self.M, cfg.C), self._f(self.M), self._f(self.M)
            ops.rows_resid_ln(a, self.Pf[lin], P[lin + '.bias'], x, y, xn, mean, rstd, cfg.eps)
            return y, (xn, mean, rstd)
        ops.gemm_nt(a, self.Wn[lin], P[lin + '.bias'], EPI_RESID, resid=x, out_f=y)
        if drop and not self.rawln:
            ops.residual_drop(y, x, cfg.J, dm.p, dm.seed_branch, dm.p_path, dm.seed_path)
        return y, None

    def _attn_fwd(self, x, pre, norm, attn, mode, need_grad, sub=0, ln=None, nxt=None, defer_proj=False):
        cfg, ops, P = self.cfg, self.ops, self.P
        M, C = self.M, cfg.C
        qkv = self._t(M, 3 * C)
        lin = f'{pre}.{attn}.qkv'
        if self.rawln:
            xn = mean = rstd = None
            ops.rows_gemm_nk_ln(x, self.Pk[lin], self.Bf[lin], self.Rs[lin], cfg.eps, qkv)
        else:
            xn, mean, rstd = self._norm_in(x, pre, norm, ln)
            ops.gemm_nt(xn, self.Wn[lin], self.Bf[lin] if self.fold else P.get(lin + '.bias'), EPI_STORE, out_t=qkv)
        dm = self._drops(pre, sub)
        o, lse = self._t(M, C), self._f(M, cfg.H)
        if self.ragged is not None and mode == MODE_TEMPORAL:
            clip_tab, n_clips, max_len = self.ragged
            ops.attn_fwd_ragged(qkv, o, lse, clip_tab, n_clips, self.B * self.Tlen, max_len, cfg.J, cfg.H, cfg.scale)
        else:
            ops.attn_fwd(qkv, o, lse, self.B, self.Tlen, cfg.J, cfg.H, cfg.scale, mode, drop=dm.attn if dm else None)
        if defer_proj:
            return x, None, None, dict(o=o, proj=f'{pre}.{attn}.proj')
        o_op = self._mm(o)
        y, ln_y = self._resid_gemm(o_op, f'{pre}.{attn}.proj', x, dm, pre, nxt)
        sv = self._saved(x, xn, mean, rstd, dm, qkv=qkv, o=o, lse=lse) if need_grad else None
        if sv is not None and self.x3 and self.x3_planes and not self.recompute:
            sv['o_op'] = o_op
        return y, sv, ln_y, None

    def _saved(self, x, xn, mean, rstd, dm, **core):
        if self.fold:
            return dict(x=None, mean=None, rstd=rstd, xn=xn, dm=dm, **core)
        return dict(x=x, mean=mean, rstd=rstd, xn=None if self.recompute else xn, dm=dm, **core)

    def _mlp_fwd(self, x, pre, norm, mlp, need_grad, sub=1, ln=None, nxt=None, pending_proj=None):
        cfg, ops, P = self.cfg, self.ops, self.P
        M, C = self.M, cfg.C
        lin = f'{pre}.{mlp}.fc1'
        if self.rawln:
            y = self._f(M, C)
            if pending_proj is not None:
                if self.Pk_proj.get(f'{pre}.{mlp}') != pending_proj['proj']:
                    raise RuntimeError(f"{pre}.{mlp}: packed with {self.Pk_proj.get(f'{pre}.{mlp}')} in front, asked to run {pending_proj['proj']}")
                ops.proj_mlp_fused_fwd(pending_proj['o'], self.Pk[f'{pre}.{mlp}'], P[pending_proj['proj'] + '.bias'], self.Bf[lin],
                                       P[f'{pre}.{mlp}.fc2.bias'], self.Rs[lin], x, y, cfg.eps)
            else:
                ops.mlp_fused_fwd(None, True, self.Pk[f'{pre}.{mlp}'], self.Bf[lin], P[f'{pre}.{mlp}.fc2.bias'], self.Rs[lin], x, y, None,
                                  cfg.eps, None, None)
            return y, None, None
        xn, mean, rstd = self._norm_in(x, pre, norm, ln)
        dm = self._drops(pre, sub)
        mlp_drop = dm is not None and dm.p > 0
        u, g = (self._t(M, cfg.hidden) if need_grad else None), (self._t(M, cfg.hidden) if mlp_drop else self._op(M, cfg.hidden))
        save_d = bool(need_grad and self.fold and self.gelu_d and self.gstream_allowed and not self.recompute and not mlp_drop
                      and lin in self.Pn and self.lnbwd_rows)
        if save_d:
            ops.gemm_nt_gelu_d(xn, self.Wn[lin], self.Bf[lin], u, g)
        else:
            ops.gemm_nt(xn, self.Wn[lin], self.Bf[lin] if self.fold else P[lin + '.bias'], EPI_GELU, out_t=u, out2_t=g)
        if mlp_drop:
            ops.dropout(g, g, dm.p, dm.seed_act)
        g = self._mm(g)
        y, ln_y = self._resid_gemm(g, f'{pre}.{mlp}.fc2', x, dm, pre, nxt)
        sv = self._saved(x, xn, mean, rstd, dm, u=None if save_d else u, d=u if save_d else None, g=None if self.recompute else g) if need_grad else None
        return y, sv, ln_y

# ... 215 lines not shown
```

motionbert_amd/hip_ops.py:

```python
from __future__ import annotations

import ctypes as C
import os
import threading
from itertools import accumulate
from typing import Dict, List, Optional

import torch

_HERE = os.path.dirname(os.path.abspath(__file__))
LIB_PATH = os.environ.get('MBX_LIB', os.path.join(_HERE, 'libmbx.so'))

MBX_F32, MBX_BF16, MBX_BF16_LO = 0, 1, 2
_DT = {torch.float32: MBX_F32, torch.bfloat16: MBX_BF16}

_vp, _i, _f, _sz, _i64p = C.c_void_p, C.c_int, C.c_float, C.c_size_t, C.c_void_p

SIGNATURES = {
    'mbx_last_error': (C.c_char_p, []),
    'mbx_version': (_i, []),
    'mbx_prep_weights': (_i, [_i64p, _i, _i, _i, _i, _vp]),
    'mbx_embed_fwd': (_i, [_vp] * 6 + [_i] * 5 + [_vp]),
    'mbx_embed_bwd_ws': (_sz, [_i] * 4),
    'mbx_embed_bwd': (_i, [_vp] * 8 + [_i] * 5 + [_vp, _vp]),
    'mbx_embed_bwd_pair': (_i, [_vp] * 9 + [_i] * 5 + [_vp, _vp]),
    'mbx_layernorm_fwd': (_i, [_vp, _vp, _vp, _f, _vp, _vp, _vp, _i, _i, _i, _vp]),
    'mbx_layernorm_bwd_ws': (_sz, [_i]),
    'mbx_layernorm_bwd': (_i, [_vp] * 11 + [_i, _i, _i, _vp, _vp]),
    'mbx_gemm_nt': (_i, [_vp, _vp, _vp, _i, _vp, _vp, _vp, _vp, _vp, _i, _i, _i, _i, _vp]),
    'mbx_gemm_tn_ws': (_sz, [_i, _i, _i]),
    'mbx_gemm_tn': (_i, [_vp, _vp, _vp, _vp, _i, _i, _i, _i, _vp, _vp]),
    'mbx_fold_norm_weights': (_i, [_i64p, _i, _i, _i, _vp]),
    'mbx_gemm_nt_dgelu_stats': (_i, [_vp] * 7 + [_i, _i, _i, _vp]),
    'mbx_gemm_nt_gelu_d': (_i, [_vp] * 5 + [_i, _i, _i, _vp]),
    'mbx_gemm_nt_mul': (_i, [_vp] * 4 + [_i, _i, _i, _vp]),
    'mbx_lnbwd_rowc': (_i, [_vp, _i, _vp, _vp, _i, _i, _vp]),
    'mbx_gemm_nt_lnbwd': (_i, [_vp] * 8 + [_i, _i, _i, _vp]),
    'mbx_gemm_nt_lnbwd_t': (_i, [_vp] * 8 + [_i, _i, _i, _vp]),
    'mbx_unfold_norm_grads_ws': (_sz, [_i, _i]),
    'mbx_unfold_norm_grads': (_i, [_vp] * 7 + [_i, _i, _vp, _vp]),
    'mbx_mlp_pack_bytes': (_sz, [_i, _i]),
    'mbx_mlp_pack_weights': (_i, [_vp, _vp, _vp, _i, _i, _vp]),
    'mbx_proj_mlp_pack_bytes': (_sz, [_i, _i]),
    'mbx_proj_mlp_pack_weights': (_i, [_vp, _vp, _vp, _vp, _i, _i, _vp]),
    'mbx_proj_mlp_fused_fwd': (_i, [_vp] * 8 + [_f, _i, _i, _i, _vp]),
    'mbx_mlp_fused_fwd': (_i, [_vp, _i] + [_vp] * 7 + [_f, _vp, _vp, _i, _i, _i, _vp]),
    'mbx_rows_pack_bytes': (_sz, [_i, _i]),
    'mbx_rows_pack_nk': (_i, [_vp, _vp, _i, _i, _vp]),
    'mbx_rows_gemm_nk': (_i, [_vp] * 7 + [_i, _i, _i, _vp]),
    'mbx_rows_gemm_nk_ln': (_i, [_vp] * 4 + [_f, _vp, _i, _i, _i, _vp]),
    'mbx_gelu_fwd': (_i, [_vp, _vp, _sz, _i, _vp]),
    'mbx_split_bf16': (_i, [_vp, _vp, _vp, _sz, _vp]),
    'mbx_gemm_nt_x3p': (_i, [_vp] * 5 + [_i] + [_vp] * 4 + [_i, _i, _i, _vp]),
    'mbx_layernorm_bwd_planes': (_i, [_vp] * 12 + [_i, _i, _vp, _vp]),
    'mbx_layernorm_fwd_planes': (_i, [_vp] * 3 + [_f] + [_vp] * 4 + [_i, _i, _vp]),
    'mbx_gemm_nt_x3': (_i, [_vp] * 5 + [_i] + [_vp] * 5 + [_i, _i, _i, _vp]),
    'mbx_gemm_tn_x3_workspace': (_sz, [_i, _i, _i]),
    'mbx_gemm_tn_x3': (_i, [_vp] * 6 + [_i, _i, _i, _vp, _vp]),
    'mbx_attn_fwd': (_i, [_vp, _vp, _vp, _i, _i, _i, _i, _i, _f, _i, _i, _vp]),
    'mbx_attn_bwd_planes': (_i, [_vp] * 6 + [_i, _i, _i, _i, _i, _f, _i, _f, C.c_uint64, _vp]),
    'mbx_attn_bwd': (_i, [_vp] * 5 + [_i, _i, _i, _i, _i, _f, _i, _i, _vp]),
    'mbx_attn_fwd_drop': (_i, [_vp, _vp, _vp, _i, _i, _i, _i, _i, _f, _i, _i, _f, C.c_uint64, _vp]),
    'mbx_attn_bwd_drop': (_i, [_vp] * 5 + [_i, _i, _i, _i, _i, _f, _i, _i, _f, C.c_uint64, _vp]),
    'mbx_attn_bwd_stats': (_i, [_vp] * 8 + [_i, _i, _i, _i, _i, _f, _i, _vp]),
    'mbx_fuse_fwd': (_i, [_vp] * 6 + [_i, _i, _vp]),
    'mbx_fuse_ln_fwd': (_i, [_vp] * 12 + [_f] + [_vp] * 2 + [_i] * 3 + [_vp]),
    'mbx_fuse_bwd_ws': (_sz, [_i]),
    'mbx_fuse_bwd': (_i, [_vp] * 11 + [_i, _i, _i, _vp, _vp]),
    'mbx_fuse_bwd_pair': (_i, [_vp] * 10 + [_i, _i, _vp, _vp]),
    'mbx_average': (_i, [_vp, _vp, _vp, _sz, _vp]),
    'mbx_average_bwd': (_i, [_vp] * 5 + [_sz, _i, _vp]),
    'mbx_head_fwd': (_i, [_vp] * 4 + [_i, _i, _i, _vp]),
    'mbx_head_bwd_ws': (_sz, [_i, _i]),
    'mbx_head_bwd': (_i, [_vp] * 6 + [_i, _i, _i, _i, _vp, _vp]),
    'mbx_tanh_bwd': (_i, [_vp, _vp, _vp, _sz, _i, _vp]),
    'mbx_pose_loss_ws': (_sz, [_i, _i]),
    'mbx_pose_loss': (_i, [_vp, _vp, _f, _f, _vp, _vp, _f, _i, _i, _i, _vp, _vp]),
    'mbx_pose_loss_full_ws': (_sz, [_i, _i]),
    'mbx_pose_loss_full': (_i, [_vp, _vp] + [_f] * 6 + [_vp, _vp, _f, _i, _i, _i, _vp, _vp]),
    'mbx_loss_2d_weighted_ws': (_sz, [_i, _i]),
    'mbx_loss_2d_weighted': (_i, [_vp, _vp, _i, _vp, _i, _vp, _vp, _f, _i, _i, _i, _vp, _vp]),
    'mbx_pool_rep_fwd': (_i, [_vp, _vp, _i, _i, _i, _i, _i, _f, C.c_uint64, _vp]),
    'mbx_tanh_pool_bwd': (_i, [_vp, _vp, _vp, _i, _i, _i, _i, _i, _f, C.c_uint64, _i, _vp]),
    'mbx_dropout': (_i, [_vp, _vp, _sz, _f, C.c_uint64, _i, _vp]),
    'mbx_residual_drop': (_i, [_vp, _vp, _sz, _i, _i, _f, C.c_uint64, _f, C.c_uint64, _vp]),
    'mbx_grad_drop': (_i, [_vp, _vp, _sz, _i, _i, _f, C.c_uint64, _f, C.c_uint64, _i, _vp]),
    'mbx_augment2d': (_i, [_vp, _vp, _i, _i, _i, _i, _vp, _vp, _vp] + [_f] * 8 + [_i, C.c_uint64, _vp]),
    'mbx_embed_fwd_tta': (_i, [_vp] * 7 + [_i] * 5 + [_vp]),
    'mbx_flip_average': (_i, [_vp, _vp, _vp, _i, _i, _i, _i, _vp]),
    'mbx_pose_errors': (_i, [_vp] * 5 + [_i] * 3 + [_vp] * 2 + [_i] * 3 + [_vp]),
    'mbx_eval_reduce_ws': (_sz, [_i, _i]),
    'mbx_eval_reduce': (_i, [_vp, _vp, _i, _vp, _i, _vp, _i, _vp, _i, _i] + [_vp] * 5),
    'mbx_supcon_loss_ws': (_sz, [_i, _i]),
    'mbx_supcon_loss': (_i, [_vp, _vp, _i, _i, _i, _f, _f, _i, _f, _vp, _vp, _vp, _vp]),
    'mbx_nn_cosine': (_i, [_vp, _vp, _i, _vp, _vp, _i, _i, _vp, _vp, _vp, _vp]),
    'mbx_rot6d_theta_fwd': (_i, [_vp, _vp, _vp, _i, _vp]),
    'mbx_rot6d_theta_bwd': (_i, [_vp, _vp, _vp, _vp, _i, _vp]),
    'mbx_mesh_param_loss_ws': (_sz, [_i]),
    'mbx_mesh_param_loss': (_i, [_vp, _vp, _i, _f, _f, _f, _f, _vp, _vp, _i, _vp, _vp]),
    'mbx_mesh_errors': (_i, [_vp] * 5 + [_i, _i, _vp]),
    'mbx_smpl_pack': (_i, [_vp, _vp, _vp, _i, _vp]),
    'mbx_smpl_fwd_ws': (_sz, [_i, _i, _i]),
    'mbx_smpl_bwd_ws': (_sz, [_i, _i, _i]),
    'mbx_smpl_fwd': (_i, [_vp] * 5 + [C.POINTER(C.c_int)] + [_vp, _vp, _i, _vp, _vp, _f, _vp, _vp, _vp, _i, _i, _vp, _sz, _vp]),
    'mbx_smpl_bwd': (_i, [_vp] * 6 + [C.POINTER(C.c_int)] + [_vp, _vp, _i, _vp, _vp, _f] + [_vp] * 5 + [_i, _i, _vp, _sz, _vp]),
    'mbx_mesh_gt_ws': (_sz, [_i, _i, _i]),
    'mbx_mesh_gt': (_i, [_vp, _vp, _vp, _vp, C.c_uint64, _f] + [_vp] * 5 + [C.POINTER(C.c_int)] + [_vp, _vp, _i, _f] + [_vp] * 5 + [_i, _i, _i, _vp, _sz, _vp]),
    'mbx_action_input': (_i, [_vp, _vp, _i, _i, _i, _i, _vp, _vp] + [_f] * 8 + [_i, C.c_uint64, _vp]),
    'mbx_motion2d_input': (_i, [_vp] * 5 + [_i, _i, _i, _vp, _vp] + [_f] * 3 + [_vp] * 3 + [_f] * 8 + [_i, C.c_uint64, _vp]),
    'mbx_amass_joints': (_i, [_vp, _vp, _i, _vp, _vp, _vp, _vp, C.POINTER(C.c_int)] + [_vp] * 4 + [_i, _i, _i, _vp, _i, _vp]),
    'mbx_xent_topk': (_i, [_vp, _vp, _i, _i, _f, _vp, _vp, _vp, _vp]),
    'mbx_wild_input_ws': (_sz, [_i, _i]),
    'mbx_wild_input': (_i, [_vp, _vp, _i, _vp, _i, _i] + [C.c_double] * 4 + [_i, _i, _vp, _vp, _vp, _sz, _vp]),
    'mbx_wild_output': (_i, [_vp, _vp, _i, _vp, _i, _i, _i, _f, C.c_double, C.c_double, _vp, _vp]),
    'mbx_wild_output_ragged': (_i, [_vp, _vp, _i, _vp, _i, _i, _i, _i, _f, C.c_double, C.c_double, _vp, _vp]),
    'mbx_attn_fwd_ragged': (_i, [_vp, _vp, _vp, _vp, _i, _i, _i, _i, _i, _i, _f, _i, _vp]),
    'mbx_embed_fwd_ragged': (_i, [_vp] * 7 + [_i] * 5 + [_vp]),
    'mbx_embed_fwd_tta_ragged': (_i, [_vp] * 8 + [_i] * 5 + [_vp]),
    'mbx_wild_mesh_ws': (_sz, [_i, _i, _i, _i]),
    'mbx_wild_mesh': (_i, [_vp] * 5 + [C.POINTER(C.c_int)] + [_vp, _vp, _i] + [_vp] * 4 + [_f, _vp] + [_i] * 4 + [_vp] * 3 + [_i, _vp, _sz, _vp]),
    'mbx_scale_fit': (_i, [_vp, _vp, _vp, _i, _i, _vp, _vp]),
    'mbx_wild_mesh_place': (_i, [_vp, _vp, _i, _vp, _vp, _i, _vp, _i, _i, _vp]),
    'mbx_render_project': (_i, [_vp, _vp, _vp, _i, _i, _i, _i, _i, _vp, _vp]),
    'mbx_render_raster_ws': (_sz, [_i, _i]),
    'mbx_render_raster': (_i, [_vp, _vp, _vp] + [_i] * 5 + [_f] * 4 + [_vp, _vp, _vp, _vp, _sz, _vp]),
    'mbx_skeleton_project': (_i, [_vp, C.POINTER(C.c_double), _i, _i, _i, _i, _vp, _vp]),
    'mbx_skeleton_raster': (_i, [_vp, _vp, _vp] + [_i] * 8 + [_vp, _vp, _vp]),
    'mbx_rows_n_pack_bytes': (_sz, [_i, _i]),
    'mbx_rows_lnbwd_t': (_i, [_vp] * 6 + [_i, _i, _i, _vp]),
    'mbx_rows_n_pack_many': (_i, [_i64p, _i, _i, _i, _vp]),
    'mbx_rows_resid_ln': (_i, [_vp] * 8 + [_f, _i, _i, _i, _vp]),
    'mbx_mfma_probe_ws': (_sz, [_i]),
    'mbx_mfma_probe': (_i, [_vp, _i, _i, C.c_uint, _vp, _vp]),
    'mbx_adamw_step': (_i, [_vp, _vp, _vp, _vp, _sz, _vp, _f, _f, _f, _f, _i, _vp]),
}


def load_library(path: str = LIB_PATH) -> C.CDLL:
    if not os.path.exists(path):
        raise RuntimeError(f'{path} not found: build it with `python -m motionbert_amd.build` '
                           '(hipcc --offload-arch=gfx950); there is no fallback implementation')
    lib = C.CDLL(path)
    for name, (res, args) in SIGNATURES.items():
        fn = getattr(lib, name)
        fn.restype, fn.argtypes = res, args
    return lib


def _p(t: Optional[torch.Tensor]):
    return None if t is None else t.data_ptr()


class HipOps:

    multi_stream = True
    grad_stream_t = True

    def __init__(self, lib: Optional[C.CDLL] = None):
        self.lib = lib or load_library()
        self._ws_cache: Dict[tuple, int] = {}
        self._desc_cache: Dict[tuple, dict] = {}
        self._desc_held: Dict[int, dict] = {}
        self.weight_cache: Dict[int, tuple] = {}
        self._lock = threading.Lock()

    def _ck(self, rc: int):
        if rc != 0:
            raise RuntimeError('libmbx: ' + self.lib.mbx_last_error().decode())

    @staticmethod
    def _stream():
        return torch.cuda.current_stream().cuda_stream

    def _ws(self, key: tuple, fn, *args, device=None) -> torch.Tensor:
        n = self._ws_cache.get(key)
# ... 104 lines not shown
            Bf[l], Rs[l] = flat_b[voff:voff + N], flat_r[voff:voff + N]
        return Wn, Wt, Bf, Rs

    def gemm_nt_dgelu_stats(self, a_t, w_t, out_t, aux_t, bias_f, rsum, part):
        M, K = a_t.shape
        N = w_t.shape[0]
        self._ck(self.lib.mbx_gemm_nt_dgelu_stats(_p(a_t), _p(w_t), _p(out_t), _p(aux_t), _p(bias_f), _p(rsum), _p(part), M, N, K, self._stream()))

    @staticmethod
    def can_gelu_d(tdtype, cfg) -> bool:
        return tdtype == torch.bfloat16 and cfg.hidden >= 256 and cfg.hidden % 8 == 0 and cfg.C % 64 == 0

    def gemm_nt_gelu_d(self, a_t, w_t, bias, out_d, out_g):
        M, K = a_t.shape
        N = w_t.shape[0]
        self._ck(self.lib.mbx_gemm_nt_gelu_d(_p(a_t), _p(w_t), _p(bias), _p(out_d), _p(out_g), M, N, K, self._stream()))

    def gemm_nt_mul(self, a_t, w_t, aux_t, out_t):
        M, K = a_t.shape
        N = w_t.shape[0]
        self._ck(self.lib.mbx_gemm_nt_mul(_p(a_t), _p(w_t), _p(aux_t), _p(out_t), M, N, K, self._stream()))

    def attn_bwd_stats(self, qkv, o, do, lse, dqkv, bias_f, rsum, part, B, T, J, H, scale, mode):
        hd = o.shape[-1] // H
        self._ck(self.lib.mbx_attn_bwd_stats(_p(qkv), _p(o), _p(do), _p(lse), _p(dqkv), _p(bias_f), _p(rsum), _p(part), B, T, J, H, hd,
                                             float(scale), int(mode), self._stream()))

    def lnbwd_rowc(self, part, rstd, rowc, C):
        nb, M = part.shape[0], part.shape[1]
        self._ck(self.lib.mbx_lnbwd_rowc(_p(part), nb, _p(rstd), _p(rowc), M, int(C), self._stream()))

    def gemm_nt_lnbwd(self, a_t, w_t, xhat, rowc, dres, extra, dx, dx_t):
        M, K = a_t.shape
        N = w_t.shape[0]
        fn = self.lib.mbx_gemm_nt_lnbwd_t if dres.dtype == torch.bfloat16 else self.lib.mbx_gemm_nt_lnbwd
        self._ck(fn(_p(a_t), _p(w_t), _p(xhat), _p(rowc), _p(dres), _p(extra), _p(dx), _p(dx_t), M, N, K, self._stream()))

    @staticmethod
    def can_fuse_mlp(tdtype, cfg) -> bool:
        return tdtype == torch.bfloat16 and cfg.C in (256, 512) and cfg.hidden % 64 == 0 and cfg.hidden <= 1536

    def mlp_pack_weights(self, w1_t, w2_t):
        hidden, Cc = w1_t.shape
        packed = torch.empty(int(self.lib.mbx_mlp_pack_bytes(Cc, hidden)), dtype=torch.uint8, device=w1_t.device)
        self._ck(self.lib.mbx_mlp_pack_weights(_p(w1_t), _p(w2_t), _p(packed), Cc, hidden, self._stream()))
        return packed

    def proj_mlp_pack_weights(self, wp_t, w1_t, w2_t):
        hidden, Cc = w1_t.shape
        packed = torch.empty(int(self.lib.mbx_proj_mlp_pack_bytes(Cc, hidden)), dtype=torch.uint8, device=w1_t.device)
        self._ck(self.lib.mbx_proj_mlp_pack_weights(_p(wp_t), _p(w1_t), _p(w2_t), _p(packed), Cc, hidden, self._stream()))
        return packed

    def proj_mlp_fused_fwd(self, o_t, packed, bp, b1, b2, rsum, resid, y, eps):
        M, Cc = resid.shape
        self._ck(self.lib.mbx_proj_mlp_fused_fwd(_p(o_t), _p(packed), _p(bp), _p(b1), _p(b2), _p(rsum), _p(resid), _p(y), float(eps), M, Cc,
                                                 b1.shape[0], self._stream()))

    def mlp_fused_fwd(self, a_t, raw_in, packed, b1, b2, rsum, resid, y, y_t, eps, mean, rstd):
        M, Cc = resid.shape
        self._ck(self.lib.mbx_mlp_fused_fwd(_p(a_t), int(bool(raw_in)), _p(packed), _p(b1), _p(b2), _p(rsum), _p(resid), _p(y), _p(y_t),
                                            float(eps), _p(mean), _p(rstd), M, Cc, b1.shape[0], self._stream()))

    def rows_pack_nk(self, w_t):
        N, K = w_t.shape
        packed = torch.empty(int(self.lib.mbx_rows_pack_bytes(N, K)), dtype=torch.uint8, device=w_t.device)
        self._ck(self.lib.mbx_rows_pack_nk(_p(w_t), _p(packed), N, K, self._stream()))
        return packed

    def rows_gemm_nk(self, a_t, packed, bias, out_t, rsum=None, mean=None, rstd=None):
        M, K = a_t.shape
        self._ck(self.lib.mbx_rows_gemm_nk(_p(a_t), _p(packed), _p(bias), _p(rsum), _p(mean), _p(rstd), _p(out_t), M, out_t.shape[1], K,
                                           self._stream()))

    def rows_gemm_nk_ln(self, x, packed, bias, rsum, eps, out_t):
        M, K = x.shape
        self._ck(self.lib.mbx_rows_gemm_nk_ln(_p(x), _p(packed), _p(bias), _p(rsum), float(eps), _p(out_t), M, out_t.shape[1], K, self._stream()))

    @staticmethod
    def can_rows_lnbwd(tdtype, cfg) -> bool:
        return (tdtype == torch.bfloat16 and cfg.C in (256, 512) and cfg.hidden % 256 == 0 and cfg.hidden >= (512 if cfg.C == 512 else 256))

    def rows_n_pack(self, w_t):
        return self.rows_n_pack_many([w_t])[0]

    def rows_n_pack_many(self, ws):
        if not ws:
            return []
        dev = ws[0].device
        N = ws[0].shape[0]
        for w in ws:
            if w.shape[0] != N or N not in (256, 512) or w.shape[1] < N or w.shape[1] % 256 or w.dtype != torch.bfloat16 or not w.is_contiguous():
                raise RuntimeError(f'rows_n_pack_many: operand {tuple(w.shape)} {w.dtype} (bf16 [N, K], one N = 256 or 512 for all, K % 256 == 0, '
                                   f'K >= N, contiguous)')
        base = ws[0].data_ptr()
        store = ws[0].untyped_storage().data_ptr()
        if any(w.untyped_storage().data_ptr() != store for w in ws):
            base = 0

        def build():
            offs = list(accumulate((N * w.shape[1] * 2 for w in ws), initial=0))
            rows = [[w.data_ptr() - base, o, w.shape[1]] for w, o in zip(ws, offs)]
            return dict(desc=torch.tensor(rows, dtype=torch.int64).to(dev), offs=offs[:-1], total=offs[-1], max_k=max(w.shape[1] for w in ws))
        key = (base == 0, N, tuple((w.data_ptr() - base, w.shape[1]) for w in ws), dev.index)
        ent = self._desc_entry('rnpack', key, build)
        flat = torch.empty(ent['total'], dtype=torch.uint8, device=dev)
        desc = ent['desc'].clone()
        desc[:, 0] += base
        desc[:, 1] += flat.data_ptr()
        self._ck(self.lib.mbx_rows_n_pack_many(desc.data_ptr(), len(ws), N, ent['max_k'], self._stream()))
        return [flat[o:o + N * w.shape[1] * 2] for w, o in zip(ws, ent['offs'])]

    def rows_lnbwd_t(self, dy_t, packed, xhat, rstd, dres_t, dx_t):
        M, K = dy_t.shape
        self._ck(self.lib.mbx_rows_lnbwd_t(_p(dy_t), _p(packed), _p(xhat), _p(rstd), _p(dres_t), _p(dx_t), M, dx_t.shape[1], K, self._stream()))

    can_rows_resid_ln = can_rows_lnbwd

    def rows_resid_ln(self, a_t, packed, bias, resid, y, xhat, mean, rstd, eps):
        M, K = a_t.shape
        self._ck(self.lib.mbx_rows_resid_ln(_p(a_t), _p(packed), _p(bias), _p(resid), _p(y), _p(xhat), _p(mean), _p(rstd), float(eps), M, y.shape[1], K,
                                            self._stream()))

    def mfma_probe(self, seconds: float = 0.25, wgs_per_cu: int = 1, device=None):
        dev = torch.device('cuda', torch.cuda.current_device()) if device is None else device
        cus = torch.cuda.get_device_properties(dev).multi_processor_count
        n_wg = cus * wgs_per_cu
        ws = torch.zeros(int(self.lib.mbx_mfma_probe_ws(n_wg)), dtype=torch.uint8, device=dev)
        flops = C.c_double(0.0)

        def run(iters):
            e0, e1 = torch.cuda.Event(enable_timing=True), torch.cuda.Event(enable_timing=True)
            e0.record()
            self._ck(self.lib.mbx_mfma_probe(_p(ws), n_wg, iters, 1234, C.byref(flops), self._stream()))
            e1.record()
            e1.synchronize()
            return e0.elapsed_time(e1)
        ms = run(20000)
        iters = max(20000, int(20000 * seconds * 1e3 / max(ms, 1e-3)))
        ms = run(iters)
        st = ws[n_wg * 1024:].view(torch.int64).view(n_wg, 2).cpu().double()
        clock = float((st[:, 0] / (st[:, 1] * 1e-8)).median()) / 1e9
        return dict(tflops=flops.value / ms / 1e9, clock_ghz=clock, ms=ms, iters=iters, wgs_per_cu=wgs_per_cu)

    def unfold_norm_grads(self, dw, db, w, gamma, beta, dgamma, dbeta):
        N, K = dw.shape
        ws = self._ws(('unf', N, K), self.lib.mbx_unfold_norm_grads_ws, N, K, device=dw.device)
        self._ck(self.lib.mbx_unfold_norm_grads(_p(dw), _p(db), _p(w), _p(gamma), _p(beta), _p(dgamma), _p(dbeta), N, K, _p(ws), self._stream()))

    def embed_fwd(self, x, w, b, pos, temp, h, B, T, J):
        self._ck(self.lib.mbx_embed_fwd(_p(x), _p(w), _p(b), _p(pos), _p(temp), _p(h), B, T, J, x.shape[-1], h.shape[-1],
                                        self._stream()))

    def embed_bwd(self, dh, x, w, dw, db, dpos, dtemp, dx, B, T, J):
        Din, Cc = x.shape[-1], dh.shape[-1]
        ws = self._ws(('emb', T, J, Din, Cc), self.lib.mbx_embed_bwd_ws, T, J, Din, Cc, device=dh.device)
        dtemp.zero_()
        self._ck(self.lib.mbx_embed_bwd(_p(dh), _p(x), _p(w), _p(dw), _p(db), _p(dpos), _p(dtemp), _p(dx), B, T, J, Din, Cc,
                                        _p(ws), self._stream()))

    def embed_bwd_pair(self, dh_a, dh_b, x, w, dw, db, dpos, dtemp, dx, B, T, J):
        Din, Cc = x.shape[-1], dh_a.shape[-1]
        ws = self._ws(('emb', T, J, Din, Cc), self.lib.mbx_embed_bwd_ws, T, J, Din, Cc, device=dh_a.device)
        dtemp.zero_()
        self._ck(self.lib.mbx_embed_bwd_pair(_p(dh_a), _p(dh_b), _p(x), _p(w), _p(dw), _p(db), _p(dpos), _p(dtemp), _p(dx), B, T, J, Din, Cc,
                                             _p(ws), self._stream()))

    layernorm_fwd_planes_ok = True

    def layernorm_fwd(self, x, g, b, eps, y_t, mean, rstd):
        M, Cc = x.shape
        if isinstance(y_t, tuple):
            self._ck(self.lib.mbx_layernorm_fwd_planes(_p(x), _p(g), _p(b), float(eps), _p(y_t[0]), _p(y_t[1]), _p(mean), _p(rstd), M, Cc,
                                                       self._stream()))
            return
        self._ck(self.lib.mbx_layernorm_fwd(_p(x), _p(g), _p(b), float(eps), _p(y_t), _p(mean), _p(rstd), M, Cc,
                                            _DT[y_t.dtype], self._stream()))

    def layernorm_bwd(self, dy_t, x, mean, rstd, g, dres, extra, dx, dx_t, dg, db):
        M, Cc = x.shape
        ws = self._ws(('lnb', Cc), self.lib.mbx_layernorm_bwd_ws, Cc, device=x.device)
        if isinstance(dx_t, tuple):
            self._ck(self.lib.mbx_layernorm_bwd_planes(_p(dy_t), _p(x), _p(mean), _p(rstd), _p(g), _p(dres), _p(extra), _p(dx), _p(dx_t[0]),
                                                       _p(dx_t[1]), _p(dg), _p(db), M, Cc, _p(ws), self._stream()))
            return
        self._ck(self.lib.mbx_layernorm_bwd(_p(dy_t), _p(x), _p(mean), _p(rstd), _p(g), _p(dres), _p(extra), _p(dx), _p(dx_t),
                                            _p(dg), _p(db), M, Cc, _DT[dy_t.dtype], _p(ws), self._stream()))

    def gelu_fwd(self, u, g):
        self._ck(self.lib.mbx_gelu_fwd(_p(u), _p(g), u.numel(), _DT[u.dtype], self._stream()))

    def split(self, t):
        hi, lo = torch.empty_like(t, dtype=torch.bfloat16), torch.empty_like(t, dtype=torch.bfloat16)
        self._ck(self.lib.mbx_split_bf16(_p(t), _p(hi), _p(lo), t.numel(), self._stream()))
        return hi, lo

    def gemm_nt(self, a_t, w_t, bias, epi, out_t=None, out2_t=None, out_f=None, resid=None, aux_t=None):
        if isinstance(a_t, tuple):
            (ah, al), (wh, wl) = a_t, w_t
            M, K = ah.shape
            N = wh.shape[0]
            if wh.shape[1] != K:
                raise RuntimeError(f'libmbx: gemm_nt_x3 operand mismatch {tuple(ah.shape)} x {tuple(wh.shape)}')
            planes = out2_t if isinstance(out2_t, tuple) else (out_t if isinstance(out_t, tuple) else None)
            if planes is not None:
                self._ck(self.lib.mbx_gemm_nt_x3p(_p(ah), _p(al), _p(wh), _p(wl), _p(bias), int(epi), _p(None if planes is out_t else out_t),
                                                  _p(planes[0]), _p(planes[1]), _p(aux_t), M, N, K, self._stream()))
                return
            self._ck(self.lib.mbx_gemm_nt_x3(_p(ah), _p(al), _p(wh), _p(wl), _p(bias), int(epi), _p(out_t), _p(out2_t), _p(out_f),
                                             _p(resid), _p(aux_t), M, N, K, self._stream()))
            return
        M, K = a_t.shape
        N = w_t.shape[0]
        if w_t.shape[1] != K or a_t.dtype != w_t.dtype:
            raise RuntimeError(f'libmbx: gemm_nt operand mismatch {tuple(a_t.shape)} {a_t.dtype} x {tuple(w_t.shape)} {w_t.dtype}')
        self._ck(self.lib.mbx_gemm_nt(_p(a_t), _p(w_t), _p(bias), int(epi), _p(out_t), _p(out2_t), _p(out_f), _p(resid),
                                      _p(aux_t), M, N, K, _DT[a_t.dtype], self._stream()))

    def gemm_tn(self, dy_t, a_t, dw, db):
        if isinstance(dy_t, tuple):
            (yh, yl), (ah, al) = dy_t, a_t
            M, N = yh.shape
            K = ah.shape[1]
            ws = self._ws(('tnx3', M, N, K), self.lib.mbx_gemm_tn_x3_workspace, M, N, K, device=yh.device)
            self._ck(self.lib.mbx_gemm_tn_x3(_p(yh), _p(yl), _p(ah), _p(al), _p(dw), _p(db), M, N, K, _p(ws), self._stream()))
            return
        M, N = dy_t.shape
        K = a_t.shape[1]
        ws = self._ws(('tn', M, N, K), self.lib.mbx_gemm_tn_ws, M, N, K, device=dy_t.device)
        self._ck(self.lib.mbx_gemm_tn(_p(dy_t), _p(a_t), _p(dw), _p(db), M, N, K, _DT[dy_t.dtype], _p(ws), self._stream()))

    def attn_fwd(self, qkv, o, lse, B, T, J, H, scale, mode, drop=None):
        hd = o.shape[-1] // H
        if drop is not None and drop[0] > 0:
            self._ck(self.lib.mbx_attn_fwd_drop(_p(qkv), _p(o), _p(lse), B, T, J, H, hd, float(scale), int(mode), _DT[qkv.dtype],
                                                float(drop[0]), int(drop[1]), self._stream()))
            return
        self._ck(self.lib.mbx_attn_fwd(_p(qkv), _p(o), _p(lse), B, T, J, H, hd, float(scale), int(mode), _DT[qkv.dtype],
                                       self._stream()))

    def attn_fwd_ragged(self, qkv, o, lse, clip_tab, n_clips, F, max_len, J, H, scale):
        if qkv.shape[0] != F * J or o.shape[0] != F * J or lse.numel() != F * J * H or qkv.shape[-1] != 3 * o.shape[-1]:
            raise RuntimeError(f'libmbx: attn_fwd_ragged needs qkv [{F * J},3C], o [{F * J},C] and lse [{F * J},{H}], got {tuple(qkv.shape)}, '
                               f'{tuple(o.shape)}, {tuple(lse.shape)}')
        if not all(t.is_contiguous() and t.device == qkv.device for t in (qkv, o, lse, clip_tab)) or o.dtype != qkv.dtype:
            raise RuntimeError('libmbx: attn_fwd_ragged needs contiguous tensors of one dtype on one device')
        self._dense('attn_fwd_ragged', torch.float32, F * J * H, qkv.device, lse=lse)
        self._dense('attn_fwd_ragged', torch.int32, None, qkv.device, clip_tab=clip_tab)
        if clip_tab.numel() < 2 * n_clips:
            raise RuntimeError(f'libmbx: attn_fwd_ragged: a table of {clip_tab.numel() // 2} rows for {n_clips} clips')
        self._ck(self.lib.mbx_attn_fwd_ragged(_p(qkv), _p(o), _p(lse), _p(clip_tab), int(n_clips), int(F), int(max_len), J, H, o.shape[-1] // H,
                                              float(scale), _DT[qkv.dtype], self._stream()))

    def attn_bwd(self, qkv, o, do, lse, dqkv, B, T, J, H, scale, mode, drop=None):
        hd = o.shape[-1] // H
        if isinstance(dqkv, tuple):
            p, seed = (float(drop[0]), int(drop[1])) if drop is not None and drop[0] > 0 else (0.0, 0)
            self._ck(self.lib.mbx_attn_bwd_planes(_p(qkv), _p(o), _p(do), _p(lse), _p(dqkv[0]), _p(dqkv[1]), B, T, J, H, hd, float(scale),
                                                  int(mode), p, seed, self._stream()))
            return
        if drop is not None and drop[0] > 0:
            self._ck(self.lib.mbx_attn_bwd_drop(_p(qkv), _p(o), _p(do), _p(lse), _p(dqkv), B, T, J, H, hd, float(scale), int(mode),
                                                _DT[qkv.dtype], float(drop[0]), int(drop[1]), self._stream()))
            return
        self._ck(self.lib.mbx_attn_bwd(_p(qkv), _p(o), _p(do), _p(lse), _p(dqkv), B, T, J, H, hd, float(scale), int(mode),
                                       _DT[qkv.dtype], self._stream()))

    def fuse_fwd(self, x_st, x_ts, w, b, out, alpha):
        M, Cc = x_st.shape
        self._ck(self.lib.mbx_fuse_fwd(_p(x_st), _p(x_ts), _p(w), _p(b), _p(out), _p(alpha), M, Cc, self._stream()))

    def fuse_ln_fwd(self, x_st, x_ts, w, b, out, alpha, g1, b1, xn1, g2, b2, xn2, eps, mean, rstd):
        M, Cc = x_st.shape
        self._ck(self.lib.mbx_fuse_ln_fwd(_p(x_st), _p(x_ts), _p(w), _p(b), _p(out), _p(alpha), _p(g1), _p(b1), _p(xn1), _p(g2), _p(b2),
                                          _p(xn2), float(eps), _p(mean), _p(rstd), M, Cc, _DT[xn1.dtype], self._stream()))

    def fuse_bwd(self, dh, x_st, x_ts, alpha, w, d_st, d_ts, d_st_t, d_ts_t, dw, db):
        M, Cc = x_st.shape
        ws = self._ws(('fub', Cc), self.lib.mbx_fuse_bwd_ws, Cc, device=dh.device)
        self._ck(self.lib.mbx_fuse_bwd(_p(dh), _p(x_st), _p(x_ts), _p(alpha), _p(w), _p(d_st), _p(d_ts), _p(d_st_t), _p(d_ts_t),
                                       _p(dw), _p(db), M, Cc, _DT[d_st_t.dtype], _p(ws), self._stream()))

    def fuse_bwd_pair(self, dh_a, dh_b, x_st, x_ts, alpha, w, d_st_t, d_ts_t, dw, db):
        M, Cc = x_st.shape
        ws = self._ws(('fub', Cc), self.lib.mbx_fuse_bwd_ws, Cc, device=x_st.device)
        self._ck(self.lib.mbx_fuse_bwd_pair(_p(dh_a), _p(dh_b), _p(x_st), _p(x_ts), _p(alpha), _p(w), _p(d_st_t), _p(d_ts_t), _p(dw), _p(db), M, Cc,
                                            _p(ws), self._stream()))

    def average(self, x_st, x_ts, out):
        self._ck(self.lib.mbx_average(_p(x_st), _p(x_ts), _p(out), x_st.numel(), self._stream()))

    def average_bwd(self, dh, d_st, d_ts, d_st_t, d_ts_t):
        self._ck(self.lib.mbx_average_bwd(_p(dh), _p(d_st), _p(d_ts), _p(d_st_t), _p(d_ts_t), dh.numel(), _DT[d_st_t.dtype],
                                          self._stream()))

    def head_fwd(self, rep, w, b, out):
        M, R = rep.shape
        self._ck(self.lib.mbx_head_fwd(_p(rep), _p(w), _p(b), _p(out), M, R, w.shape[0], self._stream()))

    def head_bwd(self, dout, rep, w, dpre_t, dw, db):
        M, R = rep.shape
        D = w.shape[0]
        ws = self._ws(('hdb', R, D), self.lib.mbx_head_bwd_ws, R, D, device=rep.device)
        self._ck(self.lib.mbx_head_bwd(_p(dout), _p(rep), _p(w), _p(dpre_t), _p(dw), _p(db), M, R, D, _DT[dpre_t.dtype], _p(ws),
                                       self._stream()))

# ... 585 lines not shown
```

Measured before the change: 585.5 clips/s.

## Fuse embedding with first layernorm, merge colsum launches, restructure embed/head backward

```diff
diff --git a/include/mbx.h b/include/mbx.h
--- a/include/mbx.h
+++ b/include/mbx.h
@@ -37,6 +37,8 @@
 
 int mbx_embed_fwd(const float* x, const float* w, const float* b, const float* pos, const float* temp,
                   float* h, int B, int T, int J, int Din, int C, void* stream);
+int mbx_embed_ln_fwd(const float* x, const float* w, const float* b, const float* pos, const float* temp, float eps, float* h,
+                     void* xhat, float* mean, float* rstd, int B, int T, int J, int Din, int C, void* stream);
 size_t mbx_embed_bwd_ws(int T, int J, int Din, int C);
 int mbx_embed_bwd(const float* dh, const float* x, const float* w, float* dw, float* db, float* dpos,
                   float* dtemp, float* dx, int B, int T, int J, int Din, int C, void* ws, void* stream);
diff --git a/motionbert_amd/csrc/elementwise.hip b/motionbert_amd/csrc/elementwise.hip
--- a/motionbert_amd/csrc/elementwise.hip
+++ b/motionbert_amd/csrc/elementwise.hip
@@ -43,14 +43,21 @@
     g_cus[dev].store(c, std::memory_order_relaxed);
     return c;
 }
-extern "C" int mbx_version(void) { return 210; }
+extern "C" int mbx_version(void) { return 220; }
 
 static inline int clamp_grid(size_t want, int cap) { return (int)(want < (size_t)cap ? (want ? want : 1) : (size_t)cap); }
 
+struct ColOut {
+    float* out[3];
+    int split0, split1, nvalid;
+};
+static inline ColOut col_out(float* o0, int ncols) { return ColOut{{o0, nullptr, nullptr}, ncols, ncols, ncols}; }
+__device__ __forceinline__ float* col_dst(const ColOut& o, int c) {
+    return c < o.split0 ? o.out[0] + c : c < o.split1 ? o.out[1] + (c - o.split0) : o.out[2] + (c - o.split1);
+}
 __device__ __forceinline__ float4 ld4(const float* p) { return *reinterpret_cast<const float4*>(p); }
 template <int CL>
-__global__ __launch_bounds__(256) void colsum4_kernel(const float* __restrict__ part, int nparts, size_t stride, int ncols,
-                                                      float* __restrict__ out0, float* __restrict__ out1, int split) {
+__global__ __launch_bounds__(256) void colsum4_kernel(const float* __restrict__ part, int nparts, size_t stride, int ncols, ColOut o) {
     constexpr int PLW = 64 / CL, PL = 4 * PLW;
     __shared__ float4 red[PL][CL];
     const int lane = threadIdx.x & 63, wave = threadIdx.x >> 6;
@@ -69,60 +76,66 @@
     }
     red[pl][cl] = (a0 + a1) + (a2 + a3);
     __syncthreads();
-    if (pl == 0 && c < ncols) {
+    if (pl == 0 && c < o.nvalid) {
         float4 t = red[0][cl];
 #pragma unroll
         for (int q = 1; q < PL; ++q) t += red[q][cl];
-        float* o = c < split ? out0 + c : out1 + (c - split);
-        if ((reinterpret_cast<uintptr_t>(o) & 15) == 0) {
-            *reinterpret_cast<float4*>(o) = t;
+        float* d = col_dst(o, c);
+        if (c + 3 < o.nvalid && (reinterpret_cast<uintptr_t>(d) & 15) == 0) {
+            *reinterpret_cast<float4*>(d) = t;
         } else {
-            o[0] = t.x; o[1] = t.y; o[2] = t.z; o[3] = t.w;
-        }
-    }
-}
-__global__ __launch_bounds__(256) void colsum_kernel(const float* __restrict__ part, int nparts, int stride, int col0,
-                                                     int ncols, float* __restrict__ out) {
-    __shared__ float red[4][64];
-    const int cl = threadIdx.x & 63, grp = threadIdx.x >> 6;
-    const int c = blockIdx.x * 64 + cl;
-    float s0 = 0.f, s1 = 0.f, s2 = 0.f, s3 = 0.f;
+            const float tv[4] = {t.x, t.y, t.z, t.w};
+#pragma unroll
+            for (int e = 0; e < 4; ++e)
+                if (c + e < o.nvalid) d[e] = tv[e];
+        }
+    }
+}
+__global__ __launch_bounds__(256) void colsum_kernel(const float* __restrict__ part, int nparts, size_t stride, int ncols, ColOut o) {
+    __shared__ float red[16][17];
+    const int cl = threadIdx.x & 15, pl = threadIdx.x >> 4;
+    const int c = blockIdx.x * 16 + cl;
+    float s[8] = {0.f, 0.f, 0.f, 0.f, 0.f, 0.f, 0.f, 0.f};
     if (c < ncols) {
-        const float* p = part + col0 + c;
-        int i = grp;
-        for (; i + 12 < nparts; i += 16) {
-            s0 += p[(size_t)i * stride];
-            s1 += p[(size_t)(i + 4) * stride];
-            s2 += p[(size_t)(i + 8) * stride];
-            s3 += p[(size_t)(i + 12) * stride];
-        }
-        for (; i < nparts; i += 4) s0 += p[(size_t)i * stride];
-    }
-    red[grp][cl] = (s0 + s1) + (s2 + s3);
+        const float* p = part + c;
+        int i = pl;
+        for (; i + 7 * 16 < nparts; i += 8 * 16) {
+            float v[8];
+#pragma unroll
+            for (int u = 0; u < 8; ++u) v[u] = p[(size_t)(i + u * 16) * stride];
+#pragma unroll
+            for (int u = 0; u < 8; ++u) s[u] += v[u];
+        }
+        for (; i < nparts; i += 16) s[0] += p[(size_t)i * stride];
+    }
+    red[pl][cl] = ((s[0] + s[1]) + (s[2] + s[3])) + ((s[4] + s[5]) + (s[6] + s[7]));
     __syncthreads();
-    if (grp == 0 && c < ncols) out[c] = (red[0][cl] + red[1][cl]) + (red[2][cl] + red[3][cl]);
+    if (pl == 0 && c < o.nvalid) {
+        float t = red[0][cl];
+#pragma unroll
+        for (int q = 1; q < 16; ++q) t += red[q][cl];
+        *col_dst(o, c) = t;
+    }
+}
+static int launch_colsum_out(const float* part, int nparts, int stride, int col0, int ncols, const ColOut& o, hipStream_t s) {
+    const bool vec = ncols % 4 == 0 && col0 % 4 == 0 && stride % 4 == 0 && o.split0 % 4 == 0 && o.split1 % 4 == 0 &&
+                     (reinterpret_cast<uintptr_t>(part + col0) & 15) == 0;
+    if (!vec) {
+        hipLaunchKernelGGL(colsum_kernel, dim3((ncols + 15) / 16), dim3(256), 0, s, part + col0, nparts, (size_t)stride, ncols, o);
+    } else if (ncols / 4 >= 64 * 512) {
+        hipLaunchKernelGGL(colsum4_kernel<64>, dim3((ncols / 4 + 63) / 64), dim3(256), 0, s, part + col0, nparts, (size_t)stride, ncols, o);
+    } else {
+        hipLaunchKernelGGL(colsum4_kernel<16>, dim3((ncols / 4 + 15) / 16), dim3(256), 0, s, part + col0, nparts, (size_t)stride, ncols, o);
+    }
+    MBX_LAUNCH_CHECK("colsum");
+    return 0;
 }
 static int launch_colsum2(const float* part, int nparts, int stride, int col0, int ncols, float* out0, float* out1, int split,
                           hipStream_t s) {
-    const bool vec = ncols % 4 == 0 && col0 % 4 == 0 && stride % 4 == 0 && split % 4 == 0 &&
-                     (reinterpret_cast<uintptr_t>(part + col0) & 15) == 0;
-    if (!vec) {
-        hipLaunchKernelGGL(colsum_kernel, dim3((split + 63) / 64), dim3(256), 0, s, part, nparts, stride, col0, split, out0);
-        if (ncols > split)
-            hipLaunchKernelGGL(colsum_kernel, dim3((ncols - split + 63) / 64), dim3(256), 0, s, part, nparts, stride, col0 + split,
-                               ncols - split, out1);
-    } else if (ncols / 4 >= 64 * 512) {
-        hipLaunchKernelGGL(colsum4_kernel<64>, dim3((ncols / 4 + 63) / 64), dim3(256), 0, s, part + col0, nparts, (size_t)stride, ncols,
-                           out0, out1, split);
-    } else {
-        hipLaunchKernelGGL(colsum4_kernel<16>, dim3((ncols / 4 + 15) / 16), dim3(256), 0, s, part + col0, nparts, (size_t)stride, ncols,
-                           out0, out1, split);
-    }
-    MBX_LAUNCH_CHECK("colsum");
-    return 0;
+    return launch_colsum_out(part, nparts, stride, col0, ncols, ColOut{{out0, out1, nullptr}, split, ncols, ncols}, s);
 }
 int mbx_launch_colsum(const float* part, int nparts, int stride, int col0, int ncols, float* out, hipStream_t s) {
-    return launch_colsum2(part, nparts, stride, col0, ncols, out, nullptr, ncols, s);
+    return launch_colsum_out(part, nparts, stride, col0, ncols, col_out(out, ncols), s);
 }
 
 struct BfLo {};
@@ -383,80 +396,91 @@
     load4<bf16_t>(dh_b + o, v);
     return make_float4(u[0] + v[0], u[1] + v[1], u[2] + v[2], u[3] + v[3]);
 }
-__global__ __launch_bounds__(256) void embed_bwd_kernel(const float* __restrict__ dh, const float* __restrict__ x,
-                                                        float* __restrict__ dtemp, float* __restrict__ part, int B, int T,
-                                                        int J, int Din, int C, const bf16_t* __restrict__ dh_a = nullptr,
-                                                        const bf16_t* __restrict__ dh_b = nullptr) {
-    __shared__ float4 red[256][1 + EMB_MAXDIN];
-    const int t = blockIdx.x;
+__device__ __forceinline__ void add4(float4& a, const float4& b) { a.x += b.x; a.y += b.y; a.z += b.z; a.w += b.w; }
+__device__ __forceinline__ void embed_bwd_walk(const float* __restrict__ dh, const bf16_t* __restrict__ dh_a, const bf16_t* __restrict__ dh_b,
+                                               const float* __restrict__ x, int B, int T, int J, int Din, int C, int t, int j, int c,
+                                               int b0, int bs, float4& ap, float4 (&aw)[EMB_MAXDIN]) {
+    for (; b0 < B; b0 += 8 * bs) {
+        float4 g[8];
+#pragma unroll
+        for (int u = 0; u < 8; ++u) {
+            const int b = min(b0 + u * bs, B - 1);
+            g[u] = embed_dh4(dh, dh_a, dh_b, (((size_t)b * T + t) * J + j) * C + c);
+        }
+#pragma unroll
+        for (int u = 0; u < 8; ++u) {
+            const int b = b0 + u * bs;
+            const float on = b < B ? 1.f : 0.f;
+            const size_t m = ((size_t)min(b, B - 1) * T + t) * J + j;
+            ap.x = fmaf(on, g[u].x, ap.x); ap.y = fmaf(on, g[u].y, ap.y); ap.z = fmaf(on, g[u].z, ap.z); ap.w = fmaf(on, g[u].w, ap.w);
+#pragma unroll
+            for (int k = 0; k < EMB_MAXDIN; ++k)
+                if (k < Din) {
+                    const float xv = on * x[m * Din + k];
+                    aw[k].x = fmaf(g[u].x, xv, aw[k].x); aw[k].y = fmaf(g[u].y, xv, aw[k].y);
+                    aw[k].z = fmaf(g[u].z, xv, aw[k].z); aw[k].w = fmaf(g[u].w, xv, aw[k].w);
+                }
+        }
+    }
+}
+template <int QB, int NS>
+__device__ __forceinline__ float4 embed_bwd_fold(float4 v, float4 (&red)[NS][QB], int sl, int ql) {
+    red[sl][ql] = v;
+    __syncthreads();
+    if (sl == 0)
+        for (int s2 = 1; s2 < NS; ++s2) add4(v, red[s2][ql]);
+    __syncthreads();
+    return v;
+}
+template <int QB, int NS>
+__global__ __launch_bounds__(QB * NS) void embed_bwd_kernel(const float* __restrict__ dh, const float* __restrict__ x,
+                                                            float* __restrict__ dtemp, float* __restrict__ part, int B, int T,
+                                                            int J, int Din, int C, const bf16_t* __restrict__ dh_a,
+                                                            const bf16_t* __restrict__ dh_b) {
+    __shared__ float4 red[NS][QB];
+    const int t = blockIdx.x, cgrp = blockIdx.y;
     const int stride = J * C + C * Din + C;
     float* prow = part + (size_t)t * stride;
-    const int nq = C / 4, ns = max(256 / nq, 1);
-    for (int q0 = 0; q0 < nq; q0 += 256) {
-        const int q = q0 + (int)threadIdx.x % min(nq, 256), sl = (int)threadIdx.x / min(nq, 256);
-        const bool act = q < nq && sl < ns;
-        const int c = q * 4;
-        float4 at = make_float4(0.f, 0.f, 0.f, 0.f), aw[EMB_MAXDIN];
-#pragma unroll
-        for (int k = 0; k < EMB_MAXDIN; ++k) aw[k] = make_float4(0.f, 0.f, 0.f, 0.f);
-        for (int j = 0; j < J; ++j) {
+    const int ql = (int)threadIdx.x % QB;
+    const int sl = QB % 64 == 0 ? __builtin_amdgcn_readfirstlane((int)threadIdx.x / QB) : (int)threadIdx.x / QB;
+    const int q = cgrp * QB + ql;
+    const bool act = q < C / 4;
+    const int c = act ? q * 4 : 0;
+    const int jfull = J - J % NS;
+    float4 at = make_float4(0.f, 0.f, 0.f, 0.f), aw[EMB_MAXDIN];
+#pragma unroll
+    for (int k = 0; k < EMB_MAXDIN; ++k) aw[k] = make_float4(0.f, 0.f, 0.f, 0.f);
+    if (act) {
+        for (int j = sl; j < jfull; j += NS) {
             float4 ap = make_float4(0.f, 0.f, 0.f, 0.f);
-            if (act) {
-                for (int b0 = sl; b0 < B; b0 += 8 * ns) {
-                    float4 g[8];
-#pragma unroll
-                    for (int u = 0; u < 8; ++u) {
-                        const int b = min(b0 + u * ns, B - 1);
-                        g[u] = embed_dh4(dh, dh_a, dh_b, (((size_t)b * T + t) * J + j) * C + c);
-                    }
-#pragma unroll
-                    for (int u = 0; u < 8; ++u) {
-                        const int b = b0 + u * ns;
-                        const float on = b < B ? 1.f : 0.f;
-                        const size_t m = ((size_t)min(b, B - 1) * T + t) * J + j;
-                        ap.x = fmaf(on, g[u].x, ap.x); ap.y = fmaf(on, g[u].y, ap.y); ap.z = fmaf(on, g[u].z, ap.z); ap.w = fmaf(on, g[u].w, ap.w);
-#pragma unroll
-                        for (int k = 0; k < EMB_MAXDIN; ++k)
-                            if (k < Din) {
-                                const float xv = on * x[m * Din + k];
-                                aw[k].x = fmaf(g[u].x, xv, aw[k].x); aw[k].y = fmaf(g[u].y, xv, aw[k].y);
-                                aw[k].z = fmaf(g[u].z, xv, aw[k].z); aw[k].w = fmaf(g[u].w, xv, aw[k].w);
-                            }
-                    }
-                }
-            }
-            red[threadIdx.x][0] = ap;
-            __syncthreads();
+            embed_bwd_walk(dh, dh_a, dh_b, x, B, T, J, Din, C, t, j, c, 0, 1, ap, aw);
+            *reinterpret_cast<float4*>(prow + (size_t)j * C + c) = ap;
+            add4(at, ap);
+        }
+    }
+    for (int j = jfull; j < J; ++j) {
+        float4 ap = make_float4(0.f, 0.f, 0.f, 0.f);
+        if (act) embed_bwd_walk(dh, dh_a, dh_b, x, B, T, J, Din, C, t, j, c, sl, NS, ap, aw);
+        ap = embed_bwd_fold<QB, NS>(ap, red, sl, ql);
+        if (act && sl == 0) {
+            *reinterpret_cast<float4*>(prow + (size_t)j * C + c) = ap;
+            add4(at, ap);
+        }
+    }
+    at = embed_bwd_fold<QB, NS>(at, red, sl, ql);
+    if (act && sl == 0) {
+        *reinterpret_cast<float4*>(dtemp + (size_t)t * C + c) = at;
+        *reinterpret_cast<float4*>(prow + (size_t)J * C + (size_t)C * Din + c) = at;
+    }
+#pragma unroll
+    for (int k = 0; k < EMB_MAXDIN; ++k)
+        if (k < Din) {
+            const float4 w4 = embed_bwd_fold<QB, NS>(aw[k], red, sl, ql);
             if (act && sl == 0) {
-                for (int s2 = 1; s2 < ns; ++s2) {
-                    const float4 o = red[threadIdx.x + s2 * nq][0];
-                    ap.x += o.x; ap.y += o.y; ap.z += o.z; ap.w += o.w;
-                }
-                *reinterpret_cast<float4*>(prow + (size_t)j * C + c) = ap;
-                at.x += ap.x; at.y += ap.y; at.z += ap.z; at.w += ap.w;
-            }
-            __syncthreads();
-        }
-#pragma unroll
-        for (int k = 0; k < EMB_MAXDIN; ++k) red[threadIdx.x][1 + k] = aw[k];
-        __syncthreads();
-        if (act && sl == 0) {
-            *reinterpret_cast<float4*>(dtemp + (size_t)t * C + c) = at;
-            *reinterpret_cast<float4*>(prow + (size_t)J * C + (size_t)C * Din + c) = at;
-#pragma unroll
-            for (int k = 0; k < EMB_MAXDIN; ++k)
-                if (k < Din) {
-                    float4 w4 = aw[k];
-                    for (int s2 = 1; s2 < ns; ++s2) {
-                        const float4 o = red[threadIdx.x + s2 * nq][1 + k];
-                        w4.x += o.x; w4.y += o.y; w4.z += o.z; w4.w += o.w;
-                    }
-                    float* d = prow + (size_t)J * C + (size_t)c * Din + k;
-                    d[0] = w4.x; d[Din] = w4.y; d[2 * Din] = w4.z; d[3 * Din] = w4.w;
-                }
-        }
-        __syncthreads();
-    }
+                float* d = prow + (size_t)J * C + (size_t)c * Din + k;
+                d[0] = w4.x; d[Din] = w4.y; d[2 * Din] = w4.z; d[3 * Din] = w4.w;
+            }
+        }
 }
 __global__ __launch_bounds__(256) void embed_bwd_dx_kernel(const float* __restrict__ dh, const float* __restrict__ w,
                                                            float* __restrict__ dx, int M, int Din, int C,
@@ -486,11 +510,13 @@
     hipStream_t s = (hipStream_t)stream;
     float* part = (float*)ws;
     const int stride = J * C + C * Din + C;
-    hipLaunchKernelGGL(embed_bwd_kernel, dim3(T), dim3(256), 0, s, dh, x, dtemp, part, B, T, J, Din, C, dh_a, dh_b);
+    const int nq = C / 4;
+#define EMBED_BWD_LAUNCH(QBV, NSV)                                                                                                  \
+    hipLaunchKernelGGL((embed_bwd_kernel<QBV, NSV>), dim3(T, (nq + QBV - 1) / QBV), dim3(QBV * NSV), 0, s, dh, x, dtemp, part, B, T, J, Din, \
+                       C, dh_a, dh_b)
+    if (nq >= 256) EMBED_BWD_LAUNCH(256, 4); else if (nq >= 128) EMBED_BWD_LAUNCH(128, 8); else EMBED_BWD_LAUNCH(64, 16);
     MBX_LAUNCH_CHECK("embed_bwd");
-    if (mbx_launch_colsum(part, T, stride, 0, J * C, dpos, s)) return 1;
-    if (mbx_launch_colsum(part, T, stride, J * C, C * Din, dw, s)) return 1;
-    if (mbx_launch_colsum(part, T, stride, J * C + C * Din, C, db, s)) return 1;
+    if (launch_colsum_out(part, T, stride, 0, stride, ColOut{{dpos, dw, db}, J * C, J * C + C * Din, stride}, s)) return 1;
     if (dx) {
         const int M = B * T * J;
         hipLaunchKernelGGL(embed_bwd_dx_kernel, dim3(clamp_grid((M + 3) / 4, 2048)), dim3(256), 0, s, dh, w, dx, M, Din, C, dh_a, dh_b);
@@ -636,6 +662,82 @@
         if (full) { LN_FWD_LAUNCH(float, true); } else { LN_FWD_LAUNCH(float, false); }
     }
     MBX_LAUNCH_CHECK("layernorm_fwd");
+    return 0;
+}
+
+template <int VPL, bool FULL>
+__device__ __forceinline__ void embed_row(const float* __restrict__ x, const float* __restrict__ pos, const float* __restrict__ temp,
+                                          const float (&wv)[VPL][4][EMBF_MAXDIN], const float (&bb)[VPL][4], int row, int T, int J, int Din,
+                                          int C, int lane, float* __restrict__ h, float4 (&raw)[VPL]) {
+    const int j = row % J, t = (row / J) % T;
+    float xv[EMBF_MAXDIN];
+#pragma unroll
+    for (int kk = 0; kk < EMBF_MAXDIN; ++kk) xv[kk] = kk < Din ? x[(size_t)row * Din + kk] : 0.f;
+    ROW_LOOP(k) {
+        const int c = ROW_C(k);
+        raw[k] = make_float4(0.f, 0.f, 0.f, 0.f);
+        if (FULL || c < C) {
+            const float4 pp = ld4(pos + (size_t)j * C + c), tt = ld4(temp + (size_t)t * C + c);
+            float a[4] = {0.f, 0.f, 0.f, 0.f};
+#pragma unroll
+            for (int kk = 0; kk < EMBF_MAXDIN; ++kk)
+                if (kk < Din) {
+#pragma unroll
+                    for (int e = 0; e < 4; ++e) a[e] = fmaf(xv[kk], wv[k][e][kk], a[e]);
+                }
+            raw[k] = make_float4(((a[0] + bb[k][0]) + pp.x) + tt.x, ((a[1] + bb[k][1]) + pp.y) + tt.y, ((a[2] + bb[k][2]) + pp.z) + tt.z,
+                                 ((a[3] + bb[k][3]) + pp.w) + tt.w);
+            *reinterpret_cast<float4*>(h + (size_t)row * C + c) = raw[k];
+        }
+    }
+}
+template <int VPL, bool FULL>
+__global__ __launch_bounds__(256) void embed_ln_fwd_kernel(const float* __restrict__ x, const float* __restrict__ w,
+                                                           const float* __restrict__ b, const float* __restrict__ pos,
+                                                           const float* __restrict__ temp, float eps, float* __restrict__ h,
+                                                           bf16_t* __restrict__ xhat, float* __restrict__ mean, float* __restrict__ rstd,
+                                                           int M, int T, int J, int Din, int C) {
+    const int lane = threadIdx.x & 63;
+    float wv[VPL][4][EMBF_MAXDIN], bb[VPL][4], g[VPL][4], bt[VPL][4];
+    ROW_LOOP(k) {
+        const int c = ROW_C(k);
+#pragma unroll
+        for (int e = 0; e < 4; ++e) {
+            g[k][e] = 1.f; bt[k][e] = 0.f; bb[k][e] = 0.f;
+#pragma unroll
+            for (int kk = 0; kk < EMBF_MAXDIN; ++kk) wv[k][e][kk] = (kk < Din && (FULL || c < C)) ? w[(size_t)(c + e) * Din + kk] : 0.f;
+        }
+        if (FULL || c < C) load4<float>(b + c, bb[k]);
+    }
+    const float invC = 1.0f / (float)C;
+    for (int row0 = (blockIdx.x * 4 + (threadIdx.x >> 6)) * 2; row0 < M; row0 += gridDim.x * 8) {
+        const int row1 = row0 + 1;
+        float4 ra[VPL], rb[VPL];
+        embed_row<VPL, FULL>(x, pos, temp, wv, bb, row0, T, J, Din, C, lane, h, ra);
+        if (row1 < M) embed_row<VPL, FULL>(x, pos, temp, wv, bb, row1, T, J, Din, C, lane, h, rb);
+        ln_fwd_row<bf16_t, VPL, FULL>(ra, g, bt, eps, invC, xhat, mean, rstd, row0, C, lane);
+        if (row1 < M) ln_fwd_row<bf16_t, VPL, FULL>(rb, g, bt, eps, invC, xhat, mean, rstd, row1, C, lane);
+    }
+}
+#define EMBED_LN_LAUNCH(VPLV, FULLV)                                                                                              \
+    hipLaunchKernelGGL((embed_ln_fwd_kernel<VPLV, FULLV>), dim3(grid), dim3(256), 0, (hipStream_t)stream, x, w, b, pos, temp, eps, h, \
+                       (bf16_t*)xhat, mean, rstd, M, T, J, Din, C)
+extern "C" int mbx_embed_ln_fwd(const float* x, const float* w, const float* b, const float* pos, const float* temp, float eps, float* h,
+                                void* xhat, float* mean, float* rstd, int B, int T, int J, int Din, int C, void* stream) {
+    MBX_CHECK_ARG(x && w && b && pos && temp && h && xhat && mean && rstd, "embed_ln_fwd: null pointer");
+    MBX_CHECK_ARG(B > 0 && T > 0 && J > 0 && Din > 0 && Din <= EMBF_MAXDIN && C > 0 && C % 4 == 0 && C <= 1024,
+                  "embed_ln_fwd: bad shape (need dim_in <= %d, C %% 4 == 0, C <= 1024)", EMBF_MAXDIN);
+    MBX_CHECK_ARG((size_t)B * T * J < ((size_t)1 << 31), "embed_ln_fwd: %zu rows do not fit a 32-bit row index", (size_t)B * T * J);
+    const int M = B * T * J;
+    const int grid = clamp_grid((M + 3) / 4, LN_BLOCKS);
+    const int vpl = vpl_for(C);
+    const bool full = C == vpl * 256;
+    switch (vpl) {
+        case 1: if (full) { EMBED_LN_LAUNCH(1, true); } else { EMBED_LN_LAUNCH(1, false); } break;
+        case 2: if (full) { EMBED_LN_LAUNCH(2, true); } else { EMBED_LN_LAUNCH(2, false); } break;
+        default: if (full) { EMBED_LN_LAUNCH(4, true); } else { EMBED_LN_LAUNCH(4, false); } break;
+    }
+    MBX_LAUNCH_CHECK("embed_ln_fwd");
     return 0;
 }
 
@@ -1245,33 +1347,54 @@
 }
 
 #define HEAD_MAXD 8
+#define HEAD_RU(VPL) ((VPL) <= 2 ? 4 : (VPL) == 4 ? 2 : 1)
+#define HEAD_BWD_RU(VPL) ((VPL) <= 2 ? 6 : HEAD_RU(VPL))
 template <int VPL>
 __global__ __launch_bounds__(256) void head_fwd_kernel(const float* __restrict__ rep, const float* __restrict__ w,
                                                        const float* __restrict__ b, float* __restrict__ out, int M, int R,
                                                        int Dout) {
+    constexpr int RU = HEAD_RU(VPL);
     const int lane = threadIdx.x & 63;
-    for (int row = blockIdx.x * 4 + (threadIdx.x >> 6); row < M; row += gridDim.x * 4) {
-        float v[VPL][4];
-        ROW_LOOP(k) {
-            const int c = ROW_C(k);
-            if (c < R) load4<float>(rep + (size_t)row * R + c, v[k]);
-        }
-        float mine = 0.f;
+    for (int row0 = (blockIdx.x * 4 + (threadIdx.x >> 6)) * RU; row0 < M; row0 += gridDim.x * 4 * RU) {
+        float v[RU][VPL][4];
+#pragma unroll
+        for (int u = 0; u < RU; ++u) {
+            const int row = min(row0 + u, M - 1);
+            ROW_LOOP(k) {
+                const int c = ROW_C(k);
+                if (c < R) load4<float>(rep + (size_t)row * R + c, v[u][k]);
+            }
+        }
+        float mine[RU];
+#pragma unroll
+        for (int u = 0; u < RU; ++u) mine[u] = 0.f;
         for (int i = 0; i < Dout; ++i) {
-            float a = 0.f;
+            float a[RU];
+#pragma unroll
+            for (int u = 0; u < RU; ++u) a[u] = 0.f;
             ROW_LOOP(k) {
                 const int c = ROW_C(k);
                 if (c < R) {
                     float ww[4];
                     load4<float>(w + (size_t)i * R + c, ww);
 #pragma unroll
-                    for (int e = 0; e < 4; ++e) a = fmaf(v[k][e], ww[e], a);
+                    for (int u = 0; u < RU; ++u)
+#pragma unroll
+                        for (int e = 0; e < 4; ++e) a[u] = fmaf(v[u][k][e], ww[e], a[u]);
                 }
             }
-            a = wave_sum(a) + b[i];
-            if (lane == i) mine = a;
-        }
-        if (lane < Dout) out[(size_t)row * Dout + lane] = mine;
+            const float bi = b[i];
+#pragma unroll
+            for (int u = 0; u < RU; ++u) {
+                const float t = wave_sum(a[u]) + bi;
+                if (lane == i) mine[u] = t;
+            }
+        }
+#pragma unroll
+        for (int u = 0; u < RU; ++u) {
+            const int row = row0 + u;
+            if (row < M && lane < Dout) out[(size_t)row * Dout + lane] = mine[u];
+        }
     }
 }
 extern "C" int mbx_head_fwd(const float* rep, const float* w, const float* b, float* out, int M, int R, int Dout,
@@ -1305,40 +1428,65 @@
                 for (int e = 0; e < 4; ++e) gw[j][k][e] = 0.f;
             }
         }
-        for (int row = blockIdx.x * 4 + wave; row < M; row += gridDim.x * 4) {
-            float dvg[DG];
-#pragma unroll
-            for (int j = 0; j < DG; ++j) dvg[j] = i0 + j < Dout ? dout[(size_t)row * Dout + i0 + j] : 0.f;
-#pragma unroll
-            for (int j = 0; j < DG; ++j) gbv[j] += dvg[j];
-            float dv[HEAD_MAXD];
+        constexpr int RU = HEAD_BWD_RU(VPL);
+        for (int row0 = (blockIdx.x * 4 + wave) * RU; row0 < M; row0 += gridDim.x * 4 * RU) {
+            float r[RU][VPL][4], dvg[RU][DG];
+            int rows[RU];
+#pragma unroll
+            for (int u = 0; u < RU; ++u) {
+                const int row = min(row0 + u, M - 1);
+                ROW_LOOP(k) {
+                    const int c = ROW_C(k);
+                    if (c < R) load4<float>(rep + (size_t)row * R + c, r[u][k]);
+                }
+#pragma unroll
+                for (int j = 0; j < DG; ++j) dvg[u][j] = i0 + j < Dout ? dout[(size_t)row * Dout + i0 + j] : 0.f;
+                rows[u] = row;
+            }
+#pragma unroll
+            for (int u = 0; u < RU; ++u) {
+                if (row0 + u < M) {
+#pragma unroll
+                    for (int j = 0; j < DG; ++j) gbv[j] += dvg[u][j];
+                    ROW_LOOP(k) {
+                        const int c = ROW_C(k);
+                        if (c < R) {
+#pragma unroll
+                            for (int j = 0; j < DG; ++j)
+#pragma unroll
+                                for (int e = 0; e < 4; ++e) gw[j][k][e] = fmaf(dvg[u][j], r[u][k][e], gw[j][k][e]);
+                        }
+                    }
+                }
+            }
             if (i0 == 0) {
-#pragma unroll
-                for (int q = 0; q < HEAD_MAXD; ++q) dv[q] = q < DG ? dvg[q < DG ? q : 0] : (q < Dout ? dout[(size_t)row * Dout + q] : 0.f);
-            }
-            ROW_LOOP(k) {
-                const int c = ROW_C(k);
-                if (c < R) {
-                    float r[4];
-                    load4<float>(rep + (size_t)row * R + c, r);
-#pragma unroll
-                    for (int j = 0; j < DG; ++j)
-#pragma unroll
-                        for (int e = 0; e < 4; ++e) gw[j][k][e] = fmaf(dvg[j], r[e], gw[j][k][e]);
-                    if (i0 == 0) {
-                        float o[4] = {0.f, 0.f, 0.f, 0.f};
+                ROW_LOOP(k) {
+                    const int c = ROW_C(k);
+                    if (c < R) {
+                        float o[RU][4];
+#pragma unroll
+                        for (int u = 0; u < RU; ++u)
+#pragma unroll
+                            for (int e = 0; e < 4; ++e) o[u][e] = 0.f;
 #pragma unroll
                         for (int q = 0; q < HEAD_MAXD; ++q) {
                             if (q < Dout) {
                                 float ww[4];
                                 load4<float>(w + (size_t)q * R + c, ww);
 #pragma unroll
-                                for (int e = 0; e < 4; ++e) o[e] = fmaf(dv[q], ww[e], o[e]);
+                                for (int u = 0; u < RU; ++u) {
+                                    const float dq = q < DG ? dvg[u][q < DG ? q : 0] : dout[(size_t)rows[u] * Dout + q];
+#pragma unroll
+                                    for (int e = 0; e < 4; ++e) o[u][e] = fmaf(dq, ww[e], o[u][e]);
+                                }
                             }
                         }
 #pragma unroll
-                        for (int e = 0; e < 4; ++e) o[e] *= (1.0f - r[e] * r[e]);
-                        store4<T>(dpre + (size_t)row * R + c, o);
+                        for (int u = 0; u < RU; ++u) {
+#pragma unroll
+                            for (int e = 0; e < 4; ++e) o[u][e] *= (1.0f - r[u][k][e] * r[u][k][e]);
+                            if (row0 + u < M) store4<T>(dpre + (size_t)(row0 + u) * R + c, o[u]);
+                        }
                     }
                 }
             }
@@ -1378,9 +1526,7 @@
         return mbx_set_error("head_bwd: unknown dtype %d", dtype);
     }
     MBX_LAUNCH_CHECK("head_bwd");
-    if (mbx_launch_colsum(part, grid, n, 0, Dout * R, dw, s)) return 1;
-    if (mbx_launch_colsum(part, grid, n, Dout * R, Dout, db, s)) return 1;
-    return 0;
+    return launch_colsum_out(part, grid, n, 0, n, ColOut{{dw, db, nullptr}, Dout * R, n, Dout * R + Dout}, s);
 }
 
 template <typename T>
diff --git a/motionbert_amd/engine.py b/motionbert_amd/engine.py
--- a/motionbert_amd/engine.py
+++ b/motionbert_amd/engine.py
@@ -308,7 +308,13 @@
         self.rawln = not need_grad and self.fold and self.drop_seed is None and self.rawln_allowed and self._can('can_fuse_mlp')
         self.prepare_weights(need_grad)
         h = self._f(M, C)
-        if ragged is not None and tta_perm is not None:
+        pos_drop = self.drop_seed is not None and cfg.drop > 0
+        ln0 = None
+        if (hasattr(ops, 'embed_ln_fwd') and self.fold and not self.rawln and not pos_drop and ragged is None and tta_perm is None
+                and self._can('can_embed_ln')):
+            ln0 = (self._t(M, C), self._f(M), self._f(M))
+            ops.embed_ln_fwd(x, P['joints_embed.weight'], P['joints_embed.bias'], P['pos_embed'], P['temp_embed'], cfg.eps, h, *ln0, B, T, J)
+        elif ragged is not None and tta_perm is not None:
             ops.embed_fwd_tta_ragged(x, tta_perm, P['joints_embed.weight'], P['joints_embed.bias'], P['pos_embed'], P['temp_embed'], frame_t, h, T, J)
         elif ragged is not None:
             ops.embed_fwd_ragged(x, P['joints_embed.weight'], P['joints_embed.bias'], P['pos_embed'], P['temp_embed'], frame_t, h, T, J)
@@ -316,7 +322,7 @@
             ops.embed_fwd_tta(x, tta_perm, P['joints_embed.weight'], P['joints_embed.bias'], P['pos_embed'], P['temp_embed'], h, B // 2, T, J)
         else:
             ops.embed_fwd(x, P['joints_embed.weight'], P['joints_embed.bias'], P['pos_embed'], P['temp_embed'], h, B, T, J)
-        if self.drop_seed is not None and cfg.drop > 0:
+        if pos_drop:
             from .dropmask import site_seed
             ops.dropout(h, h, cfg.drop, site_seed(self.drop_seed, -1, 0, 0, 1))
         saved: Dict[str, Any] = dict(x=x, levels=[], return_rep=return_rep)
@@ -324,7 +330,7 @@
         fuse_ln = cfg.att_fuse and hasattr(ops, 'fuse_ln_fwd')
         ln_st = ln_ts = ln_tail = None
         if self.fold and not self.rawln:
-            ln_st = ln_ts = self._layernorm(h, None)
+            ln_st = ln_ts = ln0 if ln0 is not None else self._layernorm(h, None)
         for i in range(cfg.depth):
             if side is not None:
                 side.wait_stream(main)
diff --git a/motionbert_amd/hip_ops.py b/motionbert_amd/hip_ops.py
--- a/motionbert_amd/hip_ops.py
+++ b/motionbert_amd/hip_ops.py
@@ -21,6 +21,7 @@
     'mbx_version': (_i, []),
     'mbx_prep_weights': (_i, [_i64p, _i, _i, _i, _i, _vp]),
     'mbx_embed_fwd': (_i, [_vp] * 6 + [_i] * 5 + [_vp]),
+    'mbx_embed_ln_fwd': (_i, [_vp] * 5 + [_f] + [_vp] * 4 + [_i] * 5 + [_vp]),
     'mbx_embed_bwd_ws': (_sz, [_i] * 4),
     'mbx_embed_bwd': (_i, [_vp] * 8 + [_i] * 5 + [_vp, _vp]),
     'mbx_embed_bwd_pair': (_i, [_vp] * 9 + [_i] * 5 + [_vp, _vp]),
@@ -431,6 +432,16 @@
         self._ck(self.lib.mbx_embed_fwd(_p(x), _p(w), _p(b), _p(pos), _p(temp), _p(h), B, T, J, x.shape[-1], h.shape[-1],
                                         self._stream()))
 
+    @staticmethod
+    def can_embed_ln(tdtype, cfg) -> bool:
+        return tdtype == torch.bfloat16 and cfg.dim_in <= 4 and cfg.C <= 1024 and cfg.C % 4 == 0
+
+    def embed_ln_fwd(self, x, w, b, pos, temp, eps, h, xhat, mean, rstd, B, T, J):
+        if xhat.dtype != torch.bfloat16:
+            raise RuntimeError('libmbx: embed_ln_fwd writes a bf16 xhat')
+        self._ck(self.lib.mbx_embed_ln_fwd(_p(x), _p(w), _p(b), _p(pos), _p(temp), float(eps), _p(h), _p(xhat), _p(mean), _p(rstd), B, T, J,
+                                           x.shape[-1], h.shape[-1], self._stream()))
+
     def embed_bwd(self, dh, x, w, dw, db, dpos, dtemp, dx, B, T, J):
         Din, Cc = x.shape[-1], dh.shape[-1]
         ws = self._ws(('emb', T, J, Din, Cc), self.lib.mbx_embed_bwd_ws, T, J, Din, Cc, device=dh.device)
```

New measurement: 591.4 clips/s (median of 6 runs). +1.0%, better.
